# cbg-ethz/LongSom

Hardware: AMD Instinct MI355X
Metric: genomic sites/s pileup+call, 10M-read BAM x 5k barcodes, 1/2/4/8 MI355X (higher is better)
Workload: dtype u32

## Files before the change

longsom_amd/csrc/lsg_api.hip:

```cpp
#include "lsg_ctx.h"
#include <cstdarg>
#include <cstring>

namespace lsg {
static thread_local char g_err[512] = "";
void set_error(const char* fmt, ...) {
    va_list ap; va_start(ap, fmt); vsnprintf(g_err, sizeof(g_err), fmt, ap); va_end(ap);
}
const char* get_error() { return g_err; }

int run_count(lsg_ctx* c, const lsg_count_params* p);
int run_fetch_counts(lsg_ctx* c, int ct, int64_t* keys, uint8_t* ref, uint32_t* counts, int64_t capacity);
int run_call(lsg_ctx* c, const lsg_call_params* p);
int run_fetch_calls(lsg_ctx* c, lsg_call* out, int64_t capacity, int candidates_only, int64_t* n_out);
int run_select_calls(lsg_ctx* c, int kind, lsg_call* dst_device, int64_t capacity, int64_t* n_out);
int run_probe(lsg_ctx* c, const PosSet& s, const char* who, const int64_t* keys, int64_t n, uint8_t* hits, int on_device);
int run_step2_allele_queries(lsg_ctx* c, int64_t* keys_out, int64_t capacity, int64_t* n_out);
int run_set_table_names(lsg_ctx* c, int32_t n_contigs, const char* contig_names, int32_t n_ct, const char* ct_names);
int run_format_table(lsg_ctx* c, int32_t table, int64_t* n_bytes);
int run_copy_table(lsg_ctx* c, int32_t table, char* dst, int64_t capacity);
int run_append_table(lsg_ctx* c, int32_t table, const char* path);
int run_free_table(lsg_ctx* c, int32_t table);
int run_step2_summary(lsg_ctx* c, int32_t n_cols, uint8_t* kinds, int64_t* n_survivor_bytes);
int run_genotype(lsg_ctx* c, const lsg_genotype_params* p, int64_t n_sites, const int64_t* site_keys, const uint8_t* alt_sym,
                 uint32_t* dp, uint32_t* alt, int on_device, int32_t max_depth, int64_t n_groups, const int64_t* group_off);
int run_cellgeno_count(lsg_ctx* c, const lsg_genotype_params* p, int32_t max_depth, int64_t n_sites, const int64_t* site_keys, const uint8_t* alt_sym,
                       const uint8_t* is_chrm, int64_t n_groups, const int64_t* group_off, double alpha2, double beta2, double pvalue);
int run_cellgeno_load_counts(lsg_ctx* c, int64_t n_sites, int32_t n_cb, const uint32_t* dp, const uint32_t* alt, const uint8_t* is_chrm, double alpha2, double beta2, double pvalue);
int run_cellgeno_fetch(lsg_ctx* c, uint32_t* dp, uint32_t* alt, int32_t* vaf4, int32_t* p4, uint8_t* status, uint8_t* bin, int64_t* n_covered, int64_t* n_pass);
int run_cellgeno_set_text(lsg_ctx* c, const lsg_cellgeno_text* t);
int run_cellgeno_filter(lsg_ctx* c, int32_t min_cells_per_mut, int32_t min_pos_cov, const uint8_t* col_int_ok, int64_t* n_rows_kept, int32_t* n_cols_kept);
int run_cellgeno_filter_fetch(lsg_ctx* c, uint8_t* row_keep, uint8_t* col_keep, int32_t* row_mut, int32_t* col_cov_kept, int32_t* col_cov_all, uint8_t* col_int);
int run_cellgeno_load_cells(lsg_ctx* c, int64_t n_sites, int32_t n_cb, const uint8_t* bin, const int32_t* vaf4);
int run_format_cell_table(lsg_ctx* c, int32_t table, int64_t* n_bytes);
int run_bnpc_load(lsg_ctx* c, int64_t n_samples, int32_t n_cells, const int32_t* assign, int32_t k_max, int32_t n_muts, const float* params);
int run_bnpc_codist(lsg_ctx* c);
int run_bnpc_fetch_dist(lsg_ctx* c, uint32_t* out, int64_t capacity);
int run_bnpc_mpear(lsg_ctx* c, int32_t n_cuts, const int32_t* labels, uint64_t* same_pairs, uint64_t* same_sim, uint64_t* dist_sum);
int run_bnpc_mean_params(lsg_ctx* c, const int32_t* final_assign, int32_t n_clusters, double* params, uint8_t* branch, int32_t* n_used);
int run_bnpc_unload(lsg_ctx* c);
int run_bnpc_linkage(lsg_ctx* c, double* Z);
int run_bnpc_cut_tree(lsg_ctx* c, int32_t n_cuts, const int32_t* n_clusters, int32_t* labels);
int run_bnpc_cluster_counts(lsg_ctx* c, int64_t* sum_over_samples);
int run_sf4(lsg_ctx* c, int64_t items, const uint32_t* k, const uint32_t* n, double al, double be, int32_t* out, double* raw);

template <class T>
static int put(lsg_ctx* c, DevBuf& buf, const T*& dst, const T* src, int64_t n, int on_device, hipStream_t st = nullptr) {
    if (n <= 0 || !src) { dst = nullptr; return 0; }
    if (src == buf.as<T>()) { dst = src; return 0; }
    if (buf.reserve((size_t)n * sizeof(T))) return -1;
    LSG_HIP(hipMemcpyAsync(buf.p, src, (size_t)n * sizeof(T), on_device ? hipMemcpyDeviceToDevice : hipMemcpyHostToDevice, st ? st : c->stream));
    dst = buf.as<T>();
    return 0;
}
static int put_ref(lsg_ctx* c, DevBuf& buf, const uint8_t*& dst, const uint8_t* src, int64_t n, int on_device) {
    if (on_device) { dst = src; return 0; }
    if (buf.reserve((size_t)n)) return -1;
    LSG_HIP(hipMemcpyAsync(buf.p, src, (size_t)n, hipMemcpyHostToDevice, c->stream));
    dst = buf.as<uint8_t>();
    return 0;
}
}

using namespace lsg;

extern "C" {

const char* lsg_last_error(void) { return get_error(); }
const char* lsg_version(void) { return "longsom_hip 0.1 (gfx950)"; }

int lsg_create(int device_id, lsg_ctx** out) {
    if (!out) { set_error("lsg_create: out is NULL"); return -2; }
    *out = nullptr;
    int n = 0;
    if (hipGetDeviceCount(&n) != hipSuccess || n <= 0) {
        set_error("lsg_create: no HIP device visible (this library has no CPU fallback)");
        return -1;
    }
    if (device_id < 0 || device_id >= n) { set_error("lsg_create: device %d out of range [0,%d)", device_id, n); return -2; }
    LSG_HIP(hipSetDevice(device_id));
    lsg_ctx* c = new lsg_ctx();
    c->device = device_id;
    { hipDeviceProp_t prop; if (hipGetDeviceProperties(&prop, device_id) == hipSuccess && prop.multiProcessorCount > 0) c->n_cus = prop.multiProcessorCount; }
    if (hipStreamCreateWithFlags(&c->copy_stream, hipStreamNonBlocking) != hipSuccess || hipEventCreateWithFlags(&c->ev_copy, hipEventDisableTiming) != hipSuccess || hipEventCreateWithFlags(&c->ev_blk, hipEventDisableTiming) != hipSuccess || hipEventCreateWithFlags(&c->ev_lpt, hipEventDisableTiming) != hipSuccess ||
        hipStreamCreateWithFlags(&c->own_stream, hipStreamNonBlocking) != hipSuccess) {
        set_error("lsg_create: hipStreamCreate failed"); delete c; return -1;
    }
    c->stream = c->own_stream;
    if (hipHostMalloc(reinterpret_cast<void**>(&c->h_pin), 4096, hipHostMallocDefault) != hipSuccess) { set_error("lsg_create: hipHostMalloc failed"); delete c; return -1; }
    for (auto& e : c->ev)
        if (hipEventCreate(&e) != hipSuccess) { set_error("lsg_create: hipEventCreate failed"); delete c; return -1; }
    for (auto& e : c->evb)
        if (hipEventCreate(&e) != hipSuccess) { set_error("lsg_create: hipEventCreate failed"); delete c; return -1; }
    *out = c;
    return 0;
}

void lsg_destroy(lsg_ctx* c) {
    if (!c) return;
    (void)hipSetDevice(c->device);
    (void)hipStreamSynchronize(c->stream);
    DevBuf* bufs[] = {&c->d_tile_base, &c->d_contig_len, &c->d_ref_ptrs, &c->d_celltype_of, &c->d_ct_rank, &c->b_read_tid, &c->b_read_pos,
                      &c->b_read_flag, &c->b_read_mapq, &c->b_read_cb, &c->b_seg_read, &c->b_seg_start, &c->b_seg_len,
                      &c->b_seg_ev_off, &c->b_events, &c->d_read_key, &c->d_read_drop, &c->d_drop_pairs, &c->d_read_adm,
                      &c->d_ne_units, &c->d_ne_mask, &c->d_ne_rowbase, &c->d_ne_rowoff,
                      &c->d_scalars, &c->d_cub_tmp, &c->d_ix_stat, &c->d_tile_cap, &c->d_tile_off, &c->d_calls, &c->d_site_off, &c->d_tail_table, &c->d_pass_list, &c->d_defer_list, &c->d_xcd_queues};
    for (auto* b : bufs) b->release();
    for (auto& b : c->d_rows) b.release();
    for (auto& b : c->ref) b.release();
    for (auto& s : c->posset) s.keys.release();
    c->alleleset.keys.release();
    for (auto& b : c->syn) b.release();
    for (auto& b : c->gen) b.release();
    (void)run_free_table(c, -1);
    c->cg.release();
    c->bnpc.release();
    c->bnpcs.release();
    c->bb.release();
    c->tab_names.release();
    for (auto& b : c->ws) b.release();
    for (auto& b : c->tm) b.release();
    for (auto& b : c->bt) b.release();
    for (auto& e : c->ev) if (e) (void)hipEventDestroy(e);
    for (auto& e : c->evb) if (e) (void)hipEventDestroy(e);
    if (c->own_stream) (void)hipStreamDestroy(c->own_stream);
    if (c->copy_stream) (void)hipStreamDestroy(c->copy_stream);
    if (c->ev_copy) (void)hipEventDestroy(c->ev_copy);
    if (c->ev_blk) (void)hipEventDestroy(c->ev_blk);
    if (c->ev_lpt) (void)hipEventDestroy(c->ev_lpt);
    if (c->h_pin) (void)hipHostFree(c->h_pin);
    delete c;
}

int lsg_unload_reads(lsg_ctx* c) {
    if (!c) { set_error("lsg_unload_reads: NULL handle"); return -2; }
    LSG_HIP(hipSetDevice(c->device));
    LSG_HIP(hipStreamSynchronize(c->stream));
    DevBuf* bufs[] = {&c->b_read_tid, &c->b_read_pos, &c->b_read_flag, &c->b_read_mapq, &c->b_read_cb, &c->b_seg_read, &c->b_seg_start, &c->b_seg_len,
                      &c->b_seg_ev_off, &c->b_events, &c->d_read_key, &c->d_read_drop, &c->d_read_adm, &c->d_ne_units, &c->d_ne_mask, &c->d_ne_rowbase, &c->d_ne_rowoff,
                      &c->d_cub_tmp, &c->d_ix_stat, &c->d_tile_cap, &c->d_tile_off, &c->d_calls, &c->d_site_off, &c->d_pass_list, &c->d_defer_list};
    for (auto* b : bufs) b->release();
    for (auto& b : c->d_rows) b.release();
    for (auto& b : c->gen) b.release();
    for (auto& b : c->ws) b.release();
    for (auto& b : c->tm) b.release();
    for (auto& b : c->bt) b.release();
    c->rd = lsg_reads{};
    lsg::drop_store(c);
    c->row_cap = 0; c->n_ne = 0; c->n_columns = 0; c->n_sites = 0; c->n_cand = 0; c->n_pass = -1;
    for (auto& n : c->n_rows) n = 0;
    return 0;
}

int lsg_set_stream(lsg_ctx* c, void* hip_stream) {
    if (!c) { set_error("lsg_set_stream: NULL handle"); return -2; }
    (void)hipStreamSynchronize(c->stream);
    c->stream = hip_stream ? reinterpret_cast<hipStream_t>(hip_stream) : c->own_stream;
    return 0;
}

int lsg_synchronize(lsg_ctx* c) {
    if (!c) { set_error("lsg_synchronize: NULL handle"); return -2; }
    LSG_HIP(hipStreamSynchronize(c->stream));
    return 0;
}

int lsg_set_contigs(lsg_ctx* c, int32_t n_contigs, const int64_t* lengths) {
    if (!c || n_contigs <= 0 || !lengths) { set_error("lsg_set_contigs: bad arguments"); return -2; }
    LSG_HIP(hipSetDevice(c->device));
    c->n_contigs = n_contigs;
    c->tab_n_contigs = 0;
    c->contig_len.assign(lengths, lengths + n_contigs);
    c->tile_base.assign(n_contigs + 1, 0);
    uint64_t t = 0;
    for (int i = 0; i < n_contigs; ++i) {
        if (lengths[i] < 0 || lengths[i] > 0x7fffffffll) { set_error("lsg_set_contigs: contig %d length %lld unsupported", i, (long long)lengths[i]); return -2; }
        c->tile_base[i] = (uint32_t)t;
        t += (uint64_t)(((lengths[i] + TILE_W - 1) / TILE_W + 1) & ~1ll);
    }
    if (t * LSG_MAX_CELLTYPES >= 0x7fffffffull) { set_error("lsg_set_contigs: genome too large (%llu tiles)", (unsigned long long)t); return -2; }
    c->tile_base[n_contigs] = (uint32_t)t;
    c->n_tiles = (uint32_t)t;
    c->tile_lo = 0; c->tile_hi = (uint32_t)t;
    lsg::drop_store(c);
    c->rd = lsg_reads{};
    for (auto& b : c->ref) b.release();
    c->ref.assign(n_contigs, DevBuf());
    c->ref_ptr.assign(n_contigs, nullptr);
    if (c->d_tile_base.reserve((size_t)(n_contigs + 1) * 4) || c->d_contig_len.reserve((size_t)n_contigs * 8) ||
        c->d_ref_ptrs.reserve((size_t)n_contigs * sizeof(void*))) return -1;
    LSG_HIP(hipMemcpyAsync(c->d_tile_base.p, c->tile_base.data(), (size_t)(n_contigs + 1) * 4, hipMemcpyHostToDevice, c->stream));
    LSG_HIP(hipMemcpyAsync(c->d_contig_len.p, c->contig_len.data(), (size_t)n_contigs * 8, hipMemcpyHostToDevice, c->stream));
    LSG_HIP(hipMemsetAsync(c->d_ref_ptrs.p, 0, (size_t)n_contigs * sizeof(void*), c->stream));
    LSG_HIP(hipStreamSynchronize(c->stream));
    c->counted = c->called = false;
    return 0;
}

int lsg_load_reference(lsg_ctx* c, int32_t tid, const uint8_t* bases, int64_t len, int32_t on_device) {
    if (!c || !bases) { set_error("lsg_load_reference: bad arguments"); return -2; }
    if (tid < 0 || tid >= c->n_contigs) { set_error("lsg_load_reference: tid %d out of range", tid); return -2; }
    if (len != c->contig_len[tid]) { set_error("lsg_load_reference: contig %d has length %lld, got %lld bases", tid, (long long)c->contig_len[tid], (long long)len); return -2; }
    LSG_HIP(hipSetDevice(c->device));
    const uint8_t* p = nullptr;
    if (put_ref(c, c->ref[tid], p, bases, len > 0 ? len : 1, on_device)) return -1;
    c->ref_ptr[tid] = p;
    LSG_HIP(hipMemcpyAsync(c->d_ref_ptrs.as<const uint8_t*>() + tid, &c->ref_ptr[tid], sizeof(void*), hipMemcpyHostToDevice, c->stream));
    LSG_HIP(hipStreamSynchronize(c->stream));
    c->counted = c->called = false;
    return 0;
}

int lsg_set_barcodes(lsg_ctx* c, const uint8_t* celltype_of, int32_t n_cb, int32_t n_celltypes) {
    if (!c || !celltype_of || n_cb <= 0) { set_error("lsg_set_barcodes: bad arguments"); return -2; }
    if (n_celltypes <= 0 || n_celltypes > LSG_MAX_CELLTYPES) { set_error("lsg_set_barcodes: n_celltypes %d not in [1,%d]", n_celltypes, LSG_MAX_CELLTYPES); return -2; }
    if (n_cb > 0x00FFFFFF) { set_error("lsg_set_barcodes: more than 2^24-1 barcodes"); return -2; }
    LSG_HIP(hipSetDevice(c->device));
    if (c->n_cb == n_cb && c->n_ct == n_celltypes && c->h_celltype_of.size() == (size_t)n_cb && memcmp(c->h_celltype_of.data(), celltype_of, (size_t)n_cb) == 0) return 0;
    c->h_celltype_of.assign(celltype_of, celltype_of + n_cb);
    if (c->d_celltype_of.reserve((size_t)n_cb)) return -1;
    LSG_HIP(hipMemcpyAsync(c->d_celltype_of.p, celltype_of, (size_t)n_cb, hipMemcpyHostToDevice, c->stream));
    {
        std::vector<uint32_t> rank((size_t)n_cb, 0u);
        for (auto& v : c->ct_size) v = 0;
        for (int32_t i = 0; i < n_cb; ++i)
            if (celltype_of[i] < n_celltypes) rank[i] = c->ct_size[celltype_of[i]]++;
        if (c->d_ct_rank.reserve((size_t)n_cb * 4)) return -1;
        LSG_HIP(hipMemcpyAsync(c->d_ct_rank.p, rank.data(), (size_t)n_cb * 4, hipMemcpyHostToDevice, c->stream));
        LSG_HIP(hipStreamSynchronize(c->stream));
    }
    LSG_HIP(hipStreamSynchronize(c->stream));
    c->n_cb = n_cb; c->n_ct = n_celltypes;
    c->max_live_reads = -1; c->max_live_exact = -1;
    c->counted = c->called = false;
    return 0;
}

int lsg_set_keep_reads(lsg_ctx* c, int32_t keep) {
    if (!c) { set_error("lsg_set_keep_reads: NULL handle"); return -2; }
    c->keep_reads = keep != 0;
    return 0;
}

int lsg_set_events_layout(lsg_ctx* c, int32_t layout) {
    if (!c || (layout != LSG_LAYOUT_COMPACT && layout != LSG_LAYOUT_PHASED)) { set_error("lsg_set_events_layout: bad arguments"); return -2; }
    c->events_layout = layout;
    return 0;
}

int lsg_set_pileup_window(lsg_ctx* c, int32_t window) {
    if (!c || window < 64) { set_error("lsg_set_pileup_window: the window must be at least 64 positions"); return -2; }
    c->plp_window = window;
    return 0;
}

int lsg_set_count_at_load(lsg_ctx* c, const lsg_count_params* params) {
    if (!c) { set_error("lsg_set_count_at_load: NULL handle"); return -2; }
    c->cal_enabled = params != nullptr;
    if (params) c->cal_params = *params;
    return 0;
}

int lsg_set_keep_unlisted(lsg_ctx* c, int32_t on) {
    if (!c) { set_error("lsg_set_keep_unlisted: NULL handle"); return -2; }
    c->keep_unlisted = on != 0;
    return 0;
}

int lsg_set_split_filters(lsg_ctx* c, int32_t max_nm, int32_t max_nh, int32_t n_trim) {
    if (!c) { set_error("lsg_set_split_filters: NULL handle"); return -2; }
    if (n_trim < 0) { set_error("lsg_set_split_filters: n_trim %d < 0", (int)n_trim); return -2; }
    c->split_max_nm = max_nm < 0 ? -1 : max_nm; c->split_max_nh = max_nh < 0 ? -1 : max_nh; c->split_n_trim = n_trim;
    return 0;
}

int lsg_get_split_reasons(lsg_ctx* c, int64_t* n, int64_t* first_ordinal) {
    if (!c || !n || !first_ordinal) { set_error("lsg_get_split_reasons: bad arguments"); return -2; }
    for (int r = 0; r < 18; ++r) { n[r] = c->split_n[r]; first_ordinal[r] = c->split_first[r]; }
    return 0;
}

int lsg_set_store_policy(lsg_ctx* c, int32_t policy) {
    if (!c) { set_error("lsg_set_store_policy: NULL handle"); return -2; }
    if (policy != LSG_STORE_KEEP && policy != LSG_STORE_SKIP_WHEN_COUNTED) { set_error("lsg_set_store_policy: unknown policy %d", (int)policy); return -2; }
    c->store_policy = policy;
    return 0;
}

int lsg_set_load_filter(lsg_ctx* c, int32_t min_mq, uint32_t flag_exclude, int32_t ignore_orphans) {
    if (!c) { set_error("lsg_set_load_filter: NULL handle"); return -2; }
    c->lf_min_mq = min_mq; c->lf_flag_exclude = flag_exclude; c->lf_ignore_orphans = ignore_orphans ? 1 : 0;
    return 0;
}

static int check_load_filter(lsg_ctx* c, const char* who, int32_t min_mq, uint32_t flag_exclude, int32_t ignore_orphans) {
    if (min_mq < c->st_min_mq || (c->st_flag_exclude & ~flag_exclude) != 0 || (c->st_ignore_orphans && !ignore_orphans)) {
        set_error("%s: these read filters (min_mq %d, flag_exclude 0x%x, ignore_orphans %d) admit reads the load filter dropped (min_mq %d, flag_exclude 0x%x, ignore_orphans %d): "
                  "load the reads again under a filter no stricter than the counts' (lsg_set_load_filter)", who, min_mq, flag_exclude, ignore_orphans,
                  c->st_min_mq, c->st_flag_exclude, c->st_ignore_orphans);
        return -2;
    }
    return 0;
}

int lsg_load_reads(lsg_ctx* c, const lsg_reads* r) {
    if (!c || !r) { set_error("lsg_load_reads: bad arguments"); return -2; }
    if (c->n_contigs <= 0) { set_error("lsg_load_reads: set the contigs first (the store is laid out over their tiles)"); return -2; }
    if (r->n_reads < 0 || r->n_segs < 0 || r->n_events < 0) { set_error("lsg_load_reads: negative sizes"); return -2; }
    if (r->n_segs >= 0xFFFFFFF0ll || r->n_reads >= (1ll << 29)) { set_error("lsg_load_reads: more than 2^32 segments or 2^29 reads; load in windows"); return -2; }
    if (r->n_events >= (1ll << 40)) { set_error("lsg_load_reads: more than 2^40 events"); return -2; }
    LSG_HIP(hipSetDevice(c->device));
    lsg::drop_store(c);
    const lsg_reads in = *r;
    c->rd = lsg_reads{};
    c->rd.n_reads = in.n_reads; c->rd.n_segs = in.n_segs; c->rd.n_events = in.n_events; c->rd.on_device = 1;
    const int d = in.on_device;
    if (in.n_reads > 0 && (!in.read_tid || !in.read_flag || !in.read_mapq || !in.read_cb)) { c->rd = lsg_reads{}; set_error("lsg_load_reads: NULL read array"); return -2; }
    if (in.n_segs > 0 && (!in.seg_read || !in.seg_start || !in.seg_len || !in.seg_ev_off)) { c->rd = lsg_reads{}; set_error("lsg_load_reads: NULL segment array"); return -2; }
    if (in.n_events > 0 && !in.events) { c->rd = lsg_reads{}; set_error("lsg_load_reads: NULL events array"); return -2; }
    hipStream_t cs = nullptr;
    if (d && !c->keep_reads) {
        LSG_HIP(hipEventRecord(c->ev_copy, c->stream));
        LSG_HIP(hipStreamWaitEvent(c->copy_stream, c->ev_copy, 0));
        cs = c->copy_stream;
    }
    if (put(c, c->b_read_tid, c->rd.read_tid, in.read_tid, in.n_reads, d, cs) ||
        put(c, c->b_read_pos, c->rd.read_pos, in.read_pos, in.n_reads, d, cs) ||
        put(c, c->b_read_flag, c->rd.read_flag, in.read_flag, in.n_reads, d, cs) ||
        put(c, c->b_read_mapq, c->rd.read_mapq, in.read_mapq, in.n_reads, d, cs) ||
        put(c, c->b_read_cb, c->rd.read_cb, in.read_cb, in.n_reads, d, cs) ||
        put(c, c->b_seg_read, c->rd.seg_read, in.seg_read, in.n_segs, d, cs) ||
        put(c, c->b_seg_start, c->rd.seg_start, in.seg_start, in.n_segs, d, cs) ||
        put(c, c->b_seg_len, c->rd.seg_len, in.seg_len, in.n_segs, d, cs)) { if (cs) (void)hipStreamSynchronize(cs); c->rd = lsg_reads{}; return -1; }
    const uint16_t* ev = in.events; const int64_t* evo = in.seg_ev_off;
    const bool staged = !d || c->keep_reads;
    if (staged && (put(c, c->b_seg_ev_off, evo, in.seg_ev_off, in.n_segs, d) || put(c, c->b_events, ev, in.events, in.n_events, d))) { c->rd = lsg_reads{}; return -1; }
    if (staged && in.events && c->hint_phased_events == (const void*)in.events) c->hint_phased_events = ev;
    const int rc = lsg::build_store(c, ev, in.n_events, evo, cs ? &in : nullptr);
    if (cs) LSG_HIP(hipStreamSynchronize(cs));
    if (rc) { c->rd = lsg_reads{}; lsg::drop_store(c); return rc; }
    if (c->keep_reads) { c->rd.events = ev; c->rd.seg_ev_off = evo; }
    else { c->b_events.release(); c->b_seg_ev_off.release(); }
    return 0;
}

int lsg_set_region(lsg_ctx* c, int32_t tid_lo, int64_t pos_lo, int32_t tid_hi, int64_t pos_hi) {
    if (!c || c->n_contigs <= 0) { set_error("lsg_set_region: set contigs first"); return -2; }
    if (tid_lo < 0 || tid_lo > c->n_contigs || tid_hi < 0 || tid_hi > c->n_contigs || (pos_lo & 63) || (pos_hi & 63) || pos_lo < 0 || pos_hi < 0) {
        set_error("lsg_set_region: bad region (positions must be multiples of 64)"); return -2;
    }
    auto tile_of = [&](int32_t tid, int64_t pos) -> uint64_t {
        if (tid >= c->n_contigs) return c->n_tiles;
        uint64_t t = (uint64_t)c->tile_base[tid] + (uint64_t)(pos >> 6);
        return t < c->tile_base[tid + 1] ? t : c->tile_base[tid + 1];
    };
    uint64_t lo = tile_of(tid_lo, pos_lo), hi = tile_of(tid_hi, pos_hi);
    if (hi < lo) { set_error("lsg_set_region: empty or inverted region"); return -2; }
    if (c->tile_lo == (uint32_t)lo && c->tile_hi == (uint32_t)hi) return 0;
    c->tile_lo = (uint32_t)lo; c->tile_hi = (uint32_t)hi;
    c->counted = c->called = false;
    return 0;
}

int lsg_pileup_count(lsg_ctx* c, const lsg_count_params* params, int64_t* n_rows, int64_t* n_columns) {
    if (!c || !params) { set_error("lsg_pileup_count: bad arguments"); return -2; }
    LSG_HIP(hipSetDevice(c->device));
    if (int rc = check_load_filter(c, "lsg_pileup_count", params->min_mq, params->flag_exclude, params->ignore_orphans)) return rc;
    const bool have = c->counted && (c->counted_at_load || c->store_skipped) && memcmp(params, &c->last_params, sizeof(*params)) == 0;
    c->counted_at_load = false;
    if (!have) { int rc = run_count(c, params); if (rc) return rc; }
    if (n_rows) for (int i = 0; i < c->n_ct; ++i) n_rows[i] = c->n_rows[i];
    if (n_columns) *n_columns = c->n_columns;
    return 0;
}

int lsg_fetch_counts(lsg_ctx* c, int32_t ct, int64_t* keys, uint8_t* ref, uint32_t* counts, int64_t capacity) {
    if (!c || !keys || !ref || !counts) { set_error("lsg_fetch_counts: bad arguments"); return -2; }
    LSG_HIP(hipSetDevice(c->device));
    return run_fetch_counts(c, ct, keys, ref, counts, capacity);
}

int64_t lsg_max_live_reads(lsg_ctx* c) {
    if (!c) { set_error("lsg_max_live_reads: bad arguments"); return -1; }
    if (hipSetDevice(c->device) != hipSuccess) { set_error("lsg_max_live_reads: hipSetDevice failed"); return -1; }
    if (lsg::live_read_bound(c)) return -1;
    return c->max_live_reads;
}

int64_t lsg_max_live_reads_exact(lsg_ctx* c) {
    if (!c) { set_error("lsg_max_live_reads_exact: bad arguments"); return -1; }
    if (hipSetDevice(c->device) != hipSuccess) { set_error("lsg_max_live_reads_exact: hipSetDevice failed"); return -1; }
    if (lsg::live_read_bound_exact(c)) return -1;
    return c->max_live_exact;
}

int64_t lsg_max_live_reads_all(lsg_ctx* c) {
    if (!c) { set_error("lsg_max_live_reads_all: bad arguments"); return -1; }
    if (hipSetDevice(c->device) != hipSuccess) { set_error("lsg_max_live_reads_all: hipSetDevice failed"); return -1; }
    if (lsg::live_read_bound_all(c)) return -1;
    return c->max_live_all;
}

int lsg_get_store_shape(lsg_ctx* c, int64_t* n_entries, int64_t* n_blocks, int64_t* n_events) {
    if (!c) { set_error("lsg_get_store_shape: NULL handle"); return -2; }
    if (n_entries) *n_entries = (int64_t)c->tm_n;
    if (n_blocks) *n_blocks = (int64_t)c->tm_nblk;
    if (n_events) *n_events = c->tm_events;
    return 0;
}

int lsg_get_build_times(lsg_ctx* c, float* ms4) {
    if (!c || !ms4) { set_error("lsg_get_build_times: bad arguments"); return -2; }
    for (int i = 0; i < 4; ++i) ms4[i] = c->build_ms[i];
    return 0;
}

int lsg_get_count_stats(lsg_ctx* c, lsg_count_stats* out) {
    if (!c || !out) { set_error("lsg_get_count_stats: bad arguments"); return -2; }
    *out = c->stats;
    return 0;
}

int lsg_get_layout_info(lsg_ctx* c, int32_t* path, double* build_ms, int64_t* store_bytes) {
    if (!c) { set_error("lsg_get_layout_info: NULL handle"); return -2; }
    if (path) *path = c->store_skipped ? (c->wsh ? 6 : c->line_loads ? 5 : 4) : c->load_was_fused ? 3 : 2;
    if (build_ms) *build_ms = c->layout_build_ms;
    if (store_bytes) {
        int64_t b = 0;
        for (auto& x : c->tm) b += (int64_t)x.cap;
        for (auto& x : c->bt) b += (int64_t)x.cap;
        for (DevBuf* x : {&c->d_tile_cap, &c->d_tile_off, &c->b_events, &c->b_seg_ev_off, &c->b_read_tid, &c->b_read_pos, &c->b_read_flag, &c->b_read_mapq, &c->b_read_cb,
                          &c->b_seg_read, &c->b_seg_start, &c->b_seg_len}) b += (int64_t)x->cap;
        b += (int64_t)c->ws[WS_SEG_INFO].cap;
        *store_bytes = b;
    }
    return 0;
}

int lsg_call_step1(lsg_ctx* c, const lsg_call_params* params, int64_t* n_sites, int64_t* n_candidates) {
    if (!c || !params) { set_error("lsg_call_step1: bad arguments"); return -2; }
    LSG_HIP(hipSetDevice(c->device));
    int rc = run_call(c, params);
    if (rc) return rc;
    if (n_sites) *n_sites = c->n_sites;
    if (n_candidates) *n_candidates = c->n_cand;
    return 0;
}

int lsg_fetch_calls(lsg_ctx* c, lsg_call* out, int64_t capacity, int32_t candidates_only, int64_t* n_out) {
    if (!c || (!out && capacity > 0)) { set_error("lsg_fetch_calls: bad arguments"); return -2; }
    LSG_HIP(hipSetDevice(c->device));
    return run_fetch_calls(c, out, capacity, candidates_only, n_out);
}

int lsg_export_calls(lsg_ctx* c, int32_t kind, void* dst_device, int64_t capacity, int64_t* n_out) {
    if (!c || kind < 0 || kind > 2) { set_error("lsg_export_calls: bad arguments"); return -2; }
    LSG_HIP(hipSetDevice(c->device));
    return run_select_calls(c, kind, reinterpret_cast<lsg_call*>(dst_device), capacity, n_out);
}

int lsg_set_table_names(lsg_ctx* c, int32_t n_contigs, const char* contig_names, int32_t n_celltypes, const char* celltype_names) {
    if (!c || n_contigs < 0 || !contig_names || !celltype_names) { set_error("lsg_set_table_names: bad arguments"); return -2; }
    LSG_HIP(hipSetDevice(c->device));
    return run_set_table_names(c, n_contigs, contig_names, n_celltypes, celltype_names);
}
int lsg_format_table(lsg_ctx* c, int32_t table, int64_t* n_bytes) {
    if (!c) { set_error("lsg_format_table: bad arguments"); return -2; }
    LSG_HIP(hipSetDevice(c->device));
    if (table >= LSG_TABLE_CELL_LONG && table <= LSG_TABLE_BNPC_VAF) return run_format_cell_table(c, table, n_bytes);
    return run_format_table(c, table, n_bytes);
}
int lsg_copy_table(lsg_ctx* c, int32_t table, char* dst_host, int64_t capacity) {
    if (!c || (!dst_host && capacity > 0) || capacity < 0) { set_error("lsg_copy_table: bad arguments"); return -2; }
    LSG_HIP(hipSetDevice(c->device));
    return run_copy_table(c, table, dst_host, capacity);
}
int lsg_append_table(lsg_ctx* c, int32_t table, const char* path) {
    if (!c || !path || !*path) { set_error("lsg_append_table: bad arguments"); return -2; }
    return run_append_table(c, table, path);
}
int lsg_step2_summary(lsg_ctx* c, int32_t n_cols, uint8_t* kinds, int64_t* n_survivor_bytes) {
    if (!c || !kinds) { set_error("lsg_step2_summary: bad arguments"); return -2; }
    LSG_HIP(hipSetDevice(c->device));
    return run_step2_summary(c, n_cols, kinds, n_survivor_bytes);
}
int lsg_free_table(lsg_ctx* c, int32_t table) {
    if (!c) { set_error("lsg_free_table: bad arguments"); return -2; }
    LSG_HIP(hipSetDevice(c->device));
    return run_free_table(c, table);
}

int lsg_load_posset(lsg_ctx* c, int32_t kind, const int64_t* keys, int64_t n, int32_t on_device) {
    if (!c || kind < 0 || kind >= 3 || n < 0 || (n > 0 && !keys)) { set_error("lsg_load_posset: bad arguments"); return -2; }
    LSG_HIP(hipSetDevice(c->device));
    PosSet& s = c->posset[kind];
    s.n = 0;
    if (n == 0) return 0;
    if (s.keys.reserve((size_t)n * 8)) return -1;
    LSG_HIP(hipMemcpyAsync(s.keys.p, keys, (size_t)n * 8, on_device ? hipMemcpyDeviceToDevice : hipMemcpyHostToDevice, c->stream));
    LSG_HIP(hipStreamSynchronize(c->stream));
    s.n = n;
    return 0;
}

int lsg_probe_posset(lsg_ctx* c, int32_t kind, const int64_t* keys, int64_t n, uint8_t* hits, int32_t on_device) {
    if (!c || kind < 0 || kind >= 3 || n < 0 || (n > 0 && (!keys || !hits))) { set_error("lsg_probe_posset: bad arguments"); return -2; }
    LSG_HIP(hipSetDevice(c->device));
    return run_probe(c, c->posset[kind], "lsg_probe_posset", keys, n, hits, on_device);
}

int lsg_load_alleleset(lsg_ctx* c, const int64_t* keys, int64_t n, int32_t on_device) {
    if (!c || (n > 0 && !keys)) { set_error("lsg_load_alleleset: bad arguments"); return -2; }
    LSG_HIP(hipSetDevice(c->device));
    PosSet& s = c->alleleset;
    s.n = 0; c->alleleset_loaded = false;
    if (n < 0) return 0;
    if (n > 0) {
        if (s.keys.reserve((size_t)n * 8)) return -1;
        LSG_HIP(hipMemcpyAsync(s.keys.p, keys, (size_t)n * 8, on_device ? hipMemcpyDeviceToDevice : hipMemcpyHostToDevice, c->stream));
        LSG_HIP(hipStreamSynchronize(c->stream));
    }
    s.n = n; c->alleleset_loaded = true;
    return 0;
}

int lsg_probe_alleleset(lsg_ctx* c, const int64_t* keys, int64_t n, uint8_t* hits, int32_t on_device) {
    if (!c || n < 0 || (n > 0 && (!keys || !hits))) { set_error("lsg_probe_alleleset: bad arguments"); return -2; }
    if (!c->alleleset_loaded) { set_error("lsg_probe_alleleset: no allele set loaded (lsg_load_alleleset)"); return -2; }
    LSG_HIP(hipSetDevice(c->device));
    return run_probe(c, c->alleleset, "lsg_probe_alleleset", keys, n, hits, on_device);
}

int lsg_step2_allele_queries(lsg_ctx* c, int64_t* keys_out, int64_t capacity, int64_t* n) {
    if (!c || !n || capacity < 0 || (capacity > 0 && !keys_out)) { set_error("lsg_step2_allele_queries: bad arguments"); return -2; }
    LSG_HIP(hipSetDevice(c->device));
    return run_step2_allele_queries(c, keys_out, capacity, n);
}

int lsg_genotype_cells(lsg_ctx* c, const lsg_genotype_params* params, int64_t n_sites, const int64_t* site_keys,
                       const uint8_t* alt_sym, uint32_t* dp, uint32_t* alt, int32_t on_device) {
    if (!c || !params) { set_error("lsg_genotype_cells: bad arguments"); return -2; }
    LSG_HIP(hipSetDevice(c->device));
    if (int rc = check_load_filter(c, "lsg_genotype_cells", params->min_mq, params->flag_exclude, params->ignore_orphans)) return rc;
    return run_genotype(c, params, n_sites, site_keys, alt_sym, dp, alt, on_device, 0, 0, nullptr);
}

int lsg_genotype_cells_grouped(lsg_ctx* c, const lsg_genotype_params* params, int32_t max_depth, int64_t n_sites, const int64_t* site_keys, const uint8_t* alt_sym,
                               int64_t n_groups, const int64_t* group_off, uint32_t* dp, uint32_t* alt, int32_t on_device) {
    if (!c || !params || n_groups < 0 || (n_groups > 0 && !group_off)) { set_error("lsg_genotype_cells_grouped: bad arguments"); return -2; }
    LSG_HIP(hipSetDevice(c->device));
    if (int rc = check_load_filter(c, "lsg_genotype_cells_grouped", params->min_mq, params->flag_exclude, params->ignore_orphans)) return rc;
    if (n_groups > 0 && (group_off[0] != 0 || group_off[n_groups] != n_sites)) { set_error("lsg_genotype_cells_grouped: the groups must cover the sites"); return -2; }
    return run_genotype(c, params, n_sites, site_keys, alt_sym, dp, alt, on_device, max_depth, n_groups, group_off);
}

int lsg_cellgeno_count(lsg_ctx* c, const lsg_genotype_params* params, int32_t max_depth, int64_t n_sites, const int64_t* site_keys, const uint8_t* alt_sym,
                       const uint8_t* is_chrm, int64_t n_groups, const int64_t* group_off, double alpha2, double beta2, double pvalue) {
    if (!c || !params || n_sites < 0 || n_groups < 0 || (n_groups > 0 && !group_off) || (n_sites > 0 && (!site_keys || !alt_sym || !is_chrm))) { set_error("lsg_cellgeno_count: bad arguments"); return -2; }
    LSG_HIP(hipSetDevice(c->device));
    if (int rc = check_load_filter(c, "lsg_cellgeno_count", params->min_mq, params->flag_exclude, params->ignore_orphans)) return rc;
    if (n_groups > 0 && (group_off[0] != 0 || group_off[n_groups] != n_sites)) { set_error("lsg_cellgeno_count: the groups must cover the sites"); return -2; }
    return run_cellgeno_count(c, params, max_depth, n_sites, site_keys, alt_sym, is_chrm, n_groups, group_off, alpha2, beta2, pvalue);
}
int lsg_cellgeno_load_counts(lsg_ctx* c, int64_t n_sites, int32_t n_cb, const uint32_t* dp, const uint32_t* alt, const uint8_t* is_chrm, double alpha2, double beta2, double pvalue) {
    if (!c || n_sites < 0 || n_cb <= 0 || (n_sites > 0 && (!dp || !alt || !is_chrm))) { set_error("lsg_cellgeno_load_counts: bad arguments"); return -2; }
    LSG_HIP(hipSetDevice(c->device));
    return run_cellgeno_load_counts(c, n_sites, n_cb, dp, alt, is_chrm, alpha2, beta2, pvalue);
}
int lsg_cellgeno_fetch(lsg_ctx* c, uint32_t* dp, uint32_t* alt, int32_t* vaf4, int32_t* p4, uint8_t* status, uint8_t* bin, int64_t* n_covered, int64_t* n_pass) {
    if (!c) { set_error("lsg_cellgeno_fetch: NULL handle"); return -2; }
    LSG_HIP(hipSetDevice(c->device));
    return run_cellgeno_fetch(c, dp, alt, vaf4, p4, status, bin, n_covered, n_pass);
}
int lsg_cellgeno_set_text(lsg_ctx* c, const lsg_cellgeno_text* text) {
    if (!c || !text) { set_error("lsg_cellgeno_set_text: bad arguments"); return -2; }
    LSG_HIP(hipSetDevice(c->device));
    return run_cellgeno_set_text(c, text);
}
int lsg_cellgeno_filter(lsg_ctx* c, int32_t min_cells_per_mut, int32_t min_pos_cov, const uint8_t* col_int_ok, int64_t* n_rows_kept, int32_t* n_cols_kept) {
    if (!c) { set_error("lsg_cellgeno_filter: NULL handle"); return -2; }
    LSG_HIP(hipSetDevice(c->device));
    return run_cellgeno_filter(c, min_cells_per_mut, min_pos_cov, col_int_ok, n_rows_kept, n_cols_kept);
}
int lsg_cellgeno_filter_fetch(lsg_ctx* c, uint8_t* row_keep, uint8_t* col_keep, int32_t* row_mut, int32_t* col_cov_kept, int32_t* col_cov_all, uint8_t* col_int) {
    if (!c) { set_error("lsg_cellgeno_filter_fetch: NULL handle"); return -2; }
    LSG_HIP(hipSetDevice(c->device));
    return run_cellgeno_filter_fetch(c, row_keep, col_keep, row_mut, col_cov_kept, col_cov_all, col_int);
}
int lsg_cellgeno_load_cells(lsg_ctx* c, int64_t n_sites, int32_t n_cb, const uint8_t* bin, const int32_t* vaf4) {
    if (!c || n_sites < 0 || n_cb <= 0 || (n_sites > 0 && (!bin || !vaf4))) { set_error("lsg_cellgeno_load_cells: bad arguments"); return -2; }
    LSG_HIP(hipSetDevice(c->device));
    return run_cellgeno_load_cells(c, n_sites, n_cb, bin, vaf4);
}

int lsg_bnpc_load_samples(lsg_ctx* c, int64_t n_samples, int32_t n_cells, const int32_t* assign, int32_t k_max, int32_t n_muts, const float* params) {
    if (!c) { set_error("lsg_bnpc_load_samples: NULL handle"); return -2; }
    LSG_HIP(hipSetDevice(c->device));
    return run_bnpc_load(c, n_samples, n_cells, assign, k_max, n_muts, params);
}

int lsg_bnpc_codist(lsg_ctx* c) {
    if (!c) { set_error("lsg_bnpc_codist: NULL handle"); return -2; }
    LSG_HIP(hipSetDevice(c->device));
    return run_bnpc_codist(c);
}

int lsg_bnpc_fetch_dist(lsg_ctx* c, uint32_t* dist, int64_t capacity) {
    if (!c) { set_error("lsg_bnpc_fetch_dist: NULL handle"); return -2; }
    LSG_HIP(hipSetDevice(c->device));
    return run_bnpc_fetch_dist(c, dist, capacity);
}

int lsg_bnpc_mpear(lsg_ctx* c, int32_t n_cuts, const int32_t* labels, uint64_t* same_pairs, uint64_t* same_sim, uint64_t* dist_sum) {
    if (!c) { set_error("lsg_bnpc_mpear: NULL handle"); return -2; }
    LSG_HIP(hipSetDevice(c->device));
    return run_bnpc_mpear(c, n_cuts, labels, same_pairs, same_sim, dist_sum);
}

int lsg_bnpc_mean_params(lsg_ctx* c, const int32_t* final_assign, int32_t n_clusters, double* params, uint8_t* branch, int32_t* n_used) {
    if (!c) { set_error("lsg_bnpc_mean_params: NULL handle"); return -2; }
    LSG_HIP(hipSetDevice(c->device));
    return run_bnpc_mean_params(c, final_assign, n_clusters, params, branch, n_used);
}

int lsg_bnpc_linkage(lsg_ctx* c, double* Z) {
    if (!c) { set_error("lsg_bnpc_linkage: NULL handle"); return -2; }
    LSG_HIP(hipSetDevice(c->device));
    return run_bnpc_linkage(c, Z);
}

int lsg_bnpc_cut_tree(lsg_ctx* c, int32_t n_cuts, const int32_t* n_clusters, int32_t* labels) {
    if (!c) { set_error("lsg_bnpc_cut_tree: NULL handle"); return -2; }
    LSG_HIP(hipSetDevice(c->device));
    return run_bnpc_cut_tree(c, n_cuts, n_clusters, labels);
}

int lsg_bnpc_cluster_counts(lsg_ctx* c, int64_t* sum_over_samples) {
    if (!c) { set_error("lsg_bnpc_cluster_counts: NULL handle"); return -2; }
    LSG_HIP(hipSetDevice(c->device));
    return run_bnpc_cluster_counts(c, sum_over_samples);
}

int lsg_bnpc_unload(lsg_ctx* c) {
    if (!c) { set_error("lsg_bnpc_unload: NULL handle"); return -2; }
    LSG_HIP(hipSetDevice(c->device));
    return run_bnpc_unload(c);
}

int lsg_betabinom_sf4(lsg_ctx* c, int64_t n_items, const uint32_t* k, const uint32_t* n, double alpha, double beta, int32_t* out_p4) {
    if (!c) { set_error("lsg_betabinom_sf4: NULL handle"); return -2; }
    LSG_HIP(hipSetDevice(c->device));
    return run_sf4(c, n_items, k, n, alpha, beta, out_p4, nullptr);
}

int lsg_betabinom_sf(lsg_ctx* c, int64_t n_items, const uint32_t* k, const uint32_t* n, double alpha, double beta, int32_t* out_p4, double* out_p) {
    if (!c || !out_p) { set_error("lsg_betabinom_sf: bad arguments"); return -2; }
    LSG_HIP(hipSetDevice(c->device));
    return run_sf4(c, n_items, k, n, alpha, beta, out_p4, out_p);
}

}
```

longsom_amd/csrc/lsg_ctx.h:

```cpp
#pragma once
#include <hip/hip_runtime.h>
#include <cstdint>
#include <cstdio>
#include <string>
#include <vector>
#include "../../include/longsom_hip.h"
#include "../../include/longsom_synth.h"

namespace lsg {

constexpr int TILE_W = 64;
constexpr int ROW_PLANES = 34;
constexpr int NCTR = 33;

constexpr int ROW_QUADS = (ROW_PLANES + 3) / 4;
constexpr uint64_t ROW_BLOCK_WORDS = (uint64_t)ROW_QUADS * 256;
constexpr uint64_t ROW_STORED_WORDS = (uint64_t)ROW_QUADS * 4;
constexpr uint32_t ROW_NARROW = 1u << 31;
constexpr uint32_t ROW_NARROW_MAX = 256;
static_assert(ROW_NARROW_MAX * 255u < (1u << 16), "a narrow row's quality sum (two planes share a word) fits 16 bits");
__host__ __device__ inline uint64_t row_word(uint64_t row, int plane) {
    return (row >> 6) * ROW_BLOCK_WORDS + (uint64_t)(plane >> 2) * 256 + (row & 63) * 4 + (uint64_t)(plane & 3);
}

void set_error(const char* fmt, ...);
const char* get_error();

#define LSG_HIP(call)                                                                          \
    do {                                                                                       \
        hipError_t e_ = (call);                                                                \
        if (e_ != hipSuccess) {                                                                \
            lsg::set_error("%s failed: %s (%s:%d)", #call, hipGetErrorString(e_), __FILE__, __LINE__); \
            return -1;                                                                         \
        }                                                                                      \
    } while (0)

struct DevBuf {
    void* p = nullptr;
    size_t cap = 0;
    int reserve(size_t bytes) {
        if (bytes <= cap) return 0;
        if (p) { (void)hipFree(p); p = nullptr; cap = 0; }
        const size_t slack = bytes / 16 < ((size_t)64 << 20) ? bytes / 16 : ((size_t)64 << 20);
        size_t want = bytes + slack + 256;
        LSG_HIP(hipMalloc(&p, want));
        cap = want;
        return 0;
    }
    void release() { if (p) (void)hipFree(p); p = nullptr; cap = 0; }
    template <class T> T* as() const { return reinterpret_cast<T*>(p); }
};

struct PosSet { DevBuf keys; int64_t n = 0; };

struct CellGeno {
    DevBuf keys, alt_sym, is_chrm, dp, alt, vaf4, p4, status, bin, n_cov, n_pass, text, scratch, filt;
    int64_t n_sites = 0; int32_t n_cb = 0; bool valid = false;
    bool cells_only = false;
    bool text_valid = false; int64_t n_long = 0, n_mat = 0; int32_t n_cols = 0, float_cells = 0;
    size_t head_off_at = 0, index_off_at = 0, label_off_at = 0, cb_off_at = 0, ct_off_at = 0, long_order_at = 0, mat_order_at = 0, col_src_at = 0,
           head_at = 0, index_at = 0, label_at = 0, cb_at = 0, ct_at = 0;
    bool filt_valid = false; int64_t n_rows_kept = 0; int32_t n_cols_kept = 0;
    size_t f_row_mut_at = 0, f_cov_kept_at = 0, f_cov_all_at = 0, f_rows_at = 0, f_cols_at = 0, f_nsel_at = 0, f_row_keep_at = 0, f_col_keep_at = 0,
           f_col_int_at = 0, f_col_ok_at = 0;
    void release() { for (DevBuf* b : {&keys, &alt_sym, &is_chrm, &dp, &alt, &vaf4, &p4, &status, &bin, &n_cov, &n_pass, &text, &scratch, &filt}) b->release(); valid = text_valid = filt_valid = false; }
};

struct Bnpc {
    DevBuf lab, raw, params, dist, cuts, sums, rank, flags, owner, cl16, idx, mean, part, ord2, small;
    DevBuf work, wsmall, rec;
    std::vector<double> Z;
    std::vector<int32_t> cut_order;
    int64_t n_samples = 0; int32_t n_cells = 0, pitch = 0, k_max = 0, n_muts = 0;
    bool valid = false, dist_valid = false, has_params = false, tree_valid = false;
    void release() {
        for (DevBuf* b : {&lab, &raw, &params, &dist, &cuts, &sums, &rank, &flags, &owner, &cl16, &idx, &mean, &part, &ord2, &small, &work, &wsmall, &rec}) b->release();
        Z = {}; cut_order = {};
        valid = dist_valid = has_params = tree_valid = false;
    }
};

struct Bnpcs {
    DevBuf one, zero, pop, seeds, lab, size, colof, live, nlive, hi, theta, L1, L0, LL, alpha, prow, n1, n0, rowml, rowb, order, keys, rec_lab, rec_sc, arena, err;
    DevBuf sm_i, sm_d, sm_c, sm_t, rec_sm;
    DevBuf rates, rec_err, err_cnt, err_out;
    DevBuf psrf, psrf_out;
    DevBuf used;
    double err_prob = 0.0, err_prior[4] = {}, mix[2] = {};
    bool learn = false, fixed_assign = false;
    double sm_prob = 0.0, sm_ratio[2] = {0.75, 0.25};
    int32_t sm_scans = 3;
    int32_t n_cells = 0, n_muts = 0, n_words = 0, n_chains = 0, steps1 = 0, k_max = 0, ll_pitch = 0, pending = -1, next_step = 0;
    int32_t test_ml_end = 0;
    int64_t arena_rows = 0;
    double p = 1.0, q = 1.0, g0 = 0.0, g1 = 0.0, dpa_prob = 0.0, betaln = 0.0;
    bool valid = false, prepared = false;
    std::vector<int32_t> h_k;
    std::vector<int64_t> h_used;
    void release() {
        for (DevBuf* b : {&one, &zero, &pop, &seeds, &lab, &size, &colof, &live, &nlive, &hi, &theta, &L1, &L0, &LL, &alpha, &prow, &n1, &n0, &rowml, &rowb, &order, &keys, &rec_lab, &rec_sc,
                          &arena, &err, &sm_i, &sm_d, &sm_c, &sm_t, &rec_sm, &rates, &rec_err, &err_cnt, &err_out, &psrf, &psrf_out, &used}) b->release();
        valid = prepared = false;
    }
};

struct Bbfit {
    DevBuf hist, tails, out, ref, tmp;
    int64_t cap = 0;
    bool valid = false;
    void release() { for (DevBuf* b : {&hist, &tails, &out, &ref, &tmp}) b->release(); valid = false; cap = 0; }
};

enum { WS_NE_NSLOT = 0, WS_NE_ACC, WS_NE_GEOM, WS_MULTI_LIST, WS_MACC, WS_EXPORT_K, WS_EXPORT_R,
       WS_EXPORT_C, WS_CALL_FLAGS, WS_CALL_SEL, WS_CALL_CANDS, WS_CALL_TASKS, WS_SEG_INFO };

constexpr uint32_t CB_MASK = 0x00FFFFFFu;
constexpr uint32_t TM_RUNSTART = 1u << 31, TM_FWD = 1u << 30, TM_WHI = 1u << 29;
constexpr uint32_t TM_PAD_S0 = CB_MASK | TM_RUNSTART;
constexpr int TM_GROUP = 4;
enum { TM_STORE = 0, TM_S0, TM_B, TM_RD, TM_META, TM_BLK_TILE, TM_BLK_OFF, TM_EXT,
       TM_JOBS, TM_NE_UNITS, TM_NE_GEOM, TM_NE_NSLOT, TM_NE_ACC, TM_MULTI, TM_CHUNKS, TM_NBUF };
struct TmJob { uint32_t e0, e1, w0, slab, nj, cnt, tile, emid, base, off; int32_t tstart, tid; };
constexpr int TM_JOB_WORDS = 12;
static_assert(sizeof(TmJob) == 4 * TM_JOB_WORDS, "TmJob layout");
constexpr uint32_t TMJ_WIDE = 1u << 31;
constexpr int TM_JOB_TGT = 3072, TM_JOB_LIMIT = 4095;

}

struct lsg_ctx;
namespace lsg {
int build_store(lsg_ctx* c, const uint16_t* events, int64_t n_events, const int64_t* seg_ev_off, const lsg_reads* src = nullptr);
int ensure_plan(lsg_ctx* c);
void drop_store(lsg_ctx* c);
int live_read_bound(lsg_ctx* c);
int live_read_bound_exact(lsg_ctx* c);
int live_read_bound_all(lsg_ctx* c);
__global__ void k_read_end(const uint32_t* seg_read, const int32_t* seg_start, const int32_t* seg_len, int64_t n_segs, int32_t* read_end);
__global__ void k_read_end_init(const int32_t* read_pos, int64_t n_reads, int32_t* read_end);
int depth_cap_drops(lsg_ctx* c, const lsg_count_params* p);
struct GatherCountSrc { const uint16_t* events; int64_t n_events; const uint64_t* key; const uint32_t* rdv; int32_t cb_bits; int32_t src_shift; int32_t wsh; };
int unit_row_offsets(lsg_ctx* c, int ct, const uint32_t** off);
int run_gather_count(lsg_ctx* c, const lsg_count_params* p, const GatherCountSrc& src, bool direct);
}

struct lsg_ctx {
    int device = 0;
    hipStream_t stream = nullptr;
    hipStream_t own_stream = nullptr;
    hipStream_t copy_stream = nullptr;
    hipEvent_t ev_copy = nullptr;
    hipEvent_t ev_blk = nullptr;
    hipEvent_t ev_lpt = nullptr;
    hipEvent_t ev[6] = {nullptr, nullptr, nullptr, nullptr, nullptr, nullptr};
    hipEvent_t evb[5] = {nullptr, nullptr, nullptr, nullptr, nullptr};

    int32_t n_contigs = 0;
    std::vector<int64_t> contig_len;
    std::vector<uint32_t> tile_base;
    uint32_t n_tiles = 0;
    uint32_t tile_lo = 0, tile_hi = 0;
    lsg::DevBuf d_tile_base, d_contig_len, d_ref_ptrs;
    std::vector<lsg::DevBuf> ref;
    std::vector<const uint8_t*> ref_ptr;

    int32_t n_cb = 0, n_ct = 0;
    lsg::DevBuf d_celltype_of, d_ct_rank;
    std::vector<uint8_t> h_celltype_of;
    uint32_t ct_size[LSG_MAX_CELLTYPES] = {0, 0, 0, 0};

    lsg_reads rd{};
    lsg::DevBuf b_read_tid, b_read_pos, b_read_flag, b_read_mapq, b_read_cb;
    lsg::DevBuf b_seg_read, b_seg_start, b_seg_len, b_seg_ev_off, b_events;
    int32_t plp_window = 50000, st_window = 50000;
    int32_t lf_min_mq = 0, lf_ignore_orphans = 0; uint32_t lf_flag_exclude = 0;
    int32_t st_min_mq = 0, st_ignore_orphans = 0; uint32_t st_flag_exclude = 0;
    bool keep_unlisted = false;
    int32_t split_max_nm = -1, split_max_nh = -1, split_n_trim = 0;
    int64_t split_n[18] = {}, split_first[18] = {};
    bool keep_reads = false;
    lsg::DevBuf d_tile_cap, d_tile_off;
    lsg::DevBuf tm[lsg::TM_NBUF];
    lsg::DevBuf bt[18];
    uint64_t tm_n = 0;
    int64_t tm_events = 0;
    uint64_t tm_np = 0;
    uint32_t tm_nblk = 0, tm_njobs = 0, tm_nchunks = 0, tm_n_ne = 0, tm_n_multi = 0, tm_n_slabs = 0, tm_n_wide = 0;
    int plan_n_ct = 0;
    int plan1_n_ct = 0;
    uint32_t plan1_tot[4] = {0, 0, 0, 0};
    uint32_t plan_misc[2] = {0, 0};
    uint32_t* d_plan_misc = nullptr;
    bool cal_enabled = false; lsg_count_params cal_params{};
    bool counted_at_load = false;
    bool load_was_fused = false;
    bool tm_valid = false;
    int32_t store_policy = 0;
    bool store_skipped = false;
    double layout_build_ms = 0;
    float build_ms[4] = {0, 0, 0, 0};
    int64_t max_live_reads = -1;
    int64_t max_live_all = -1;
    int32_t wsh = 0;
    int32_t events_layout = 0;
    const void* hint_phased_events = nullptr;
    bool src_phased = false;
    bool line_loads = false;
    int64_t max_live_exact = -1;
    lsg::DevBuf d_read_drop;
    lsg::DevBuf d_drop_pairs; int64_t n_drop_pairs = 0;
    lsg::DevBuf d_read_adm;
    bool has_drops = false;
    int64_t n_depth_dropped = 0;

    lsg::DevBuf d_read_key;
    lsg::DevBuf d_ne_units, d_ne_mask, d_ne_rowbase, d_ne_rowoff, d_scalars, d_cub_tmp, d_ix_stat;
    lsg::DevBuf d_rows[LSG_MAX_CELLTYPES];
    uint64_t row_cap = 0;
    uint32_t arena = 256;
    uint32_t n_ne = 0;
    int64_t n_rows[LSG_MAX_CELLTYPES] = {0, 0, 0, 0};
    int64_t n_columns = 0;
    lsg_count_params last_params{};
    lsg_count_stats stats{};
    bool counted = false;

    lsg::DevBuf d_calls, d_site_off, d_tail_table;
    double tail_table_key[4] = {0, 0, 0, 0}; bool tail_table_valid = false;
    int64_t n_sites = 0, n_cand = 0, n_pass = -1;
    lsg::DevBuf d_pass_list, d_defer_list, d_xcd_queues;
    uint32_t call_tasks_per_site = 1;
    bool called = false;

    lsg::DevBuf tab_keys[LSG_MAX_CELLTYPES], tab_refs[LSG_MAX_CELLTYPES], tab_rows[LSG_MAX_CELLTYPES], tab_names, tab_scratch, tab_scratch2;
    int32_t tab_scratch_table = -1; int64_t tab_scratch_rows = 0;
    uint64_t tab_rows_serial[LSG_MAX_CELLTYPES] = {0, 0, 0, 0};
    uint64_t count_serial = 0;
    lsg::DevBuf tab_text[LSG_TABLE_SLOTS];
    int64_t tab_bytes[LSG_TABLE_SLOTS];
    lsg_ctx() { for (auto& b : tab_bytes) b = -1; }
    int32_t tab_n_contigs = 0, tab_n_ct = 0; uint32_t tab_ct_off_at = 0, tab_order_at = 0, tab_ct_txt_at = 0, tab_contig_txt_at = 0;

    lsg::CellGeno cg;

    lsg::Bnpc bnpc;
    lsg::Bnpcs bnpcs;
    lsg::Bbfit bb;

    lsg::PosSet posset[3];
    lsg::PosSet alleleset; bool alleleset_loaded = false;
    lsg::DevBuf syn[12];
    lsg::DevBuf gen[10];
    lsg::DevBuf ws[16];
    int n_cus = 256;
    unsigned long long* h_pin = nullptr;
    uint32_t n_multi = 0;
};
```

longsom_amd/csrc/store.hip:

```cpp
#include "lsg_ctx.h"
#include <hipcub/hipcub.hpp>
#include <chrono>
#include <cstdio>
#include <cstdlib>
#include <utility>

namespace lsg {

constexpr uint32_t KEY_INVALID = 0xFFFFFFFFu;

constexpr uint32_t RV_WHI = 1u << 29, RV_SEGFIRST = 1u << 30, RV_FWD = 1u << 31, RV_READ = RV_WHI - 1u;
__host__ __device__ __forceinline__ uint64_t sort_key(uint32_t cb, uint32_t first, uint32_t nev1, uint64_t src, int cb_bits, int wsh = 0) {
    return (uint64_t)cb | ((uint64_t)(first | (nev1 << (6 + wsh))) << cb_bits) | (src << (cb_bits + 12 + 2 * wsh));
}

struct BuildArgs {
    int64_t n_reads, n_segs, n_events;
    const int32_t* read_tid; const uint16_t* read_flag; const uint8_t* read_mapq; const int32_t* read_cb;
    const uint32_t* seg_read; const int32_t* seg_start; const int32_t* seg_len; const int64_t* seg_ev_off;
    const uint32_t* tile_base; const int64_t* contig_len;
    int32_t n_contigs; uint32_t n_tiles;
    uint2* seg_info;
    uint32_t* tile_cap;
    uint32_t* cursor;
    uint64_t* key; uint32_t* rdv;
    int32_t cb_bits;
    unsigned long long* qhead;
    int32_t lf_min_mq, lf_ignore_orphans; uint32_t lf_flag_exclude;
    uint32_t* bad;
    unsigned long long* n_ev;
    int32_t* span_diff;
    int32_t* cap_diff;
    int32_t window;
    int32_t wsh;
    int32_t src_shift;
};

__device__ __forceinline__ int64_t win_edge_after(int64_t x, int32_t W) { return 1 + (int64_t)W * (int64_t)((x >= 1 ? (uint32_t)(x - 1) / (uint32_t)W : 0u) + 1u); }
__device__ __forceinline__ int64_t win_edge_in_tile(int64_t tstart, int32_t W) {
    const int64_t b = win_edge_after(tstart, W);
    return b < tstart + TILE_W ? b : -1;
}

constexpr int SEG_THREADS = 256, SEG_U = 4, SEG_H = 2048, SEG_MAX_SINCE = 6;
__global__ __launch_bounds__(SEG_THREADS) void k_seg_static(BuildArgs a) {
    __shared__ uint32_t hkey[SEG_H];
    __shared__ int32_t hval[SEG_H];
    __shared__ unsigned long long s_ev;
    __shared__ uint32_t s_new, s_flush;
    for (int i = threadIdx.x; i < SEG_H; i += SEG_THREADS) { hkey[i] = KEY_INVALID; hval[i] = 0; }
    if (threadIdx.x == 0) { s_ev = 0; s_new = 0; s_flush = 0; }
    auto slot = [&](uint32_t t) -> int {
        uint32_t h = (t * 2654435761u) >> 21;
        for (int tries = 0; tries < 16; ++tries) {
            const uint32_t prev = atomicCAS(&hkey[h], KEY_INVALID, t);
            if (prev == KEY_INVALID) { atomicAdd(&s_new, 1u); return (int)h; }
            if (prev == t) return (int)h;
            h = (h + 1) & (SEG_H - 1);
        }
        return -1;
    };
    auto mark = [&](uint32_t t, int32_t v) { const int h = slot(t); if (h >= 0) atomicAdd(&hval[h], v); else atomicAdd(a.span_diff + t, v); };
    auto mark_cap = [&](uint32_t t, int32_t v) { const int h = slot(t); if (h >= 0) atomicAdd(&hval[h], v * 65536); else atomicAdd(a.cap_diff + t, v); };
    unsigned long long n_ev = 0;
    bool unphased = false;
    constexpr int64_t BATCH = (int64_t)SEG_THREADS * SEG_U;
    const int64_t n_batches = (a.n_segs + BATCH - 1) / BATCH;
    const int64_t per_wg = (n_batches + gridDim.x - 1) / gridDim.x;
    const int64_t b_lo = (int64_t)blockIdx.x * per_wg, b_hi = b_lo + per_wg < n_batches ? b_lo + per_wg : n_batches;
    const int64_t last_seg = a.n_segs - 1;
    int since = 0;
    __syncthreads();
    for (int64_t bt = b_lo; bt < b_hi; ++bt) {
        int64_t sg[SEG_U], st_[SEG_U], ln_[SEG_U], of_[SEG_U]; uint32_t rd_[SEG_U], rp_[SEG_U], rn_[SEG_U]; bool in_[SEG_U];
#pragma unroll
        for (int u = 0; u < SEG_U; ++u) {
            sg[u] = bt * BATCH + (int64_t)u * SEG_THREADS + threadIdx.x;
            in_[u] = sg[u] < a.n_segs;
            const int64_t si = in_[u] ? sg[u] : last_seg;
            rd_[u] = a.seg_read[si]; st_[u] = a.seg_start[si]; ln_[u] = a.seg_len[si]; of_[u] = a.seg_ev_off[si];
            rp_[u] = a.seg_read[si > 0 ? si - 1 : 0]; rn_[u] = a.seg_read[si < last_seg ? si + 1 : last_seg];
        }
        int32_t tid_[SEG_U], cb_[SEG_U]; uint32_t flag_[SEG_U], mq_[SEG_U];
#pragma unroll
        for (int u = 0; u < SEG_U; ++u) {
            const int64_t ri = (int64_t)rd_[u] < a.n_reads ? (int64_t)rd_[u] : 0;
            tid_[u] = a.read_tid[ri]; cb_[u] = a.read_cb[ri]; flag_[u] = a.read_flag[ri]; mq_[u] = (uint32_t)a.read_mapq[ri];
        }
        int64_t clen_[SEG_U]; uint32_t tb_[SEG_U], te_[SEG_U];
#pragma unroll
        for (int u = 0; u < SEG_U; ++u) {
            const int ti = tid_[u] >= 0 && tid_[u] < a.n_contigs ? tid_[u] : 0;
            clen_[u] = a.contig_len[ti]; tb_[u] = a.tile_base[ti]; te_[u] = a.tile_base[ti + 1];
        }
#pragma unroll
        for (int u = 0; u < SEG_U; ++u) {
        const int64_t s = sg[u];
        uint32_t edge_tile = KEY_INVALID;
        if (in_[u]) {
            const uint32_t r = rd_[u];
            uint32_t key = KEY_INVALID, tb = 0;
            if ((int64_t)r >= a.n_reads) atomicOr(a.bad, 2u);
            else {
                const int64_t st = st_[u], ln = ln_[u], o = of_[u];
                const int32_t tid = tid_[u], cb = cb_[u];
                const bool on_contig = tid >= 0 && tid < a.n_contigs;
                if (ln > 0 && (o < 0 || o + ln > a.n_events)) atomicOr(a.bad, 1u);
                else {
                    const uint32_t flag = flag_[u];
                    bool pool = (int)mq_[u] >= a.lf_min_mq && (flag & a.lf_flag_exclude) == 0;
                    if (pool && a.lf_ignore_orphans && (flag & 1u) && !(flag & 2u)) pool = false;
                    if (pool && on_contig && cb >= 0 && (uint32_t)cb < CB_MASK && !(st < 0 || ln <= 0 || st + ln > clen_[u])) {
                        key = (uint32_t)cb | (((flag >> 4) & 1u) << 24);
                        tb = tb_[u];
                        n_ev += (unsigned long long)ln;
                        unphased |= ((o - st) & (int64_t)((64 << a.wsh) - 1)) != 0;
                        mark_cap((tb + ((uint32_t)st >> 6)) >> a.wsh, 1);
                        mark_cap(((tb + ((uint32_t)(st + ln - 1) >> 6)) >> a.wsh) + 1, -1);
                        int nb = 0;
                        for (int64_t b = win_edge_after(st, a.window); b < st + ln; b += a.window) {
                            if ((b & (int64_t)((64 << a.wsh) - 1)) == 0) continue;
                            const uint32_t t = (tb + (uint32_t)(b >> 6)) >> a.wsh;
                            if (nb++ == 0) edge_tile = t;
                            else { atomicAdd(a.cap_diff + t, 1); atomicAdd(a.cap_diff + t + 1, -1); }
                        }
                    }
                }
                if (a.span_diff && on_contig && cb >= 0) {
                    const bool first = s == 0 || rp_[u] != r, last = s + 1 == a.n_segs || rn_[u] != r;
                    const uint32_t t0 = tb_[u], te = te_[u];
                    if ((first || last) && te > t0) {
                        int64_t b = st < 0 ? 0 : st, e = st + (ln > 0 ? ln : 0);
                        if (e < 0) e = 0;
                        if (first) { uint32_t t = t0 + (uint32_t)(b >> 6); if (t >= te) t = te - 1; mark(t >> a.wsh, 1); }
                        if (last) { uint32_t t = t0 + (uint32_t)(e >> 6); if (t >= te) t = te - 1; mark((t >> a.wsh) + 1, -1); }
                    }
                }
            }
            a.seg_info[s] = make_uint2(key, tb);
        }
        for (unsigned long long todo = __ballot(edge_tile != KEY_INVALID); todo;) {
            const uint32_t lt = (uint32_t)__shfl((int)edge_tile, __ffsll((long long)todo) - 1);
            const unsigned long long same = __ballot(edge_tile == lt);
            if ((threadIdx.x & 63) == (unsigned)(__ffsll((long long)todo) - 1)) { const int n = __popcll(same); atomicAdd(a.cap_diff + lt, n); atomicAdd(a.cap_diff + lt + 1, -n); }
            todo &= ~same;
        }
        }
        ++since;
        __syncthreads();
        if (threadIdx.x == 0) {
            s_flush = (bt + 1 == b_hi || s_new > SEG_H / 2 || since >= SEG_MAX_SINCE) ? 1u : 0u;
            if (s_flush) s_new = 0;
        }
        __syncthreads();
        if (s_flush) {
            since = 0;
            for (int i = threadIdx.x; i < SEG_H; i += SEG_THREADS)
                if (hkey[i] != KEY_INVALID) {
                    const int32_t w = hval[i], v = (int32_t)(int16_t)(w & 0xffff), cp = (w - v) >> 16;
                    if (v != 0) atomicAdd(a.span_diff + hkey[i], v);
                    if (cp != 0) atomicAdd(a.cap_diff + hkey[i], cp);
                    hkey[i] = KEY_INVALID; hval[i] = 0;
                }
            __syncthreads();
        }
    }
    for (int o = 32; o > 0; o >>= 1) n_ev += __shfl_down(n_ev, o);
    __syncthreads();
    if ((threadIdx.x & 63) == 0 && n_ev) atomicAdd(&s_ev, n_ev);
    __syncthreads();
    if (threadIdx.x == 0 && s_ev) atomicAdd(a.n_ev, s_ev);
    if (__syncthreads_or(unphased ? 1 : 0) && threadIdx.x == 0) atomicOr(a.bad, 4u);
}

constexpr int BIN_THREADS = 256;
constexpr int BIN_TPR = 8;
constexpr int BIN_H = 4096;
constexpr int BIN_SUPER = 16;
constexpr int BIN_MAXI = 32;
constexpr uint32_t BIN_FILL = BIN_H * 5 / 8;

template <class OP>
__device__ __forceinline__ uint32_t wave_reduce_last(uint32_t v, OP op) {
    v = op(v, (uint32_t)__builtin_amdgcn_update_dpp(0, (int)v, 0x111, 0xf, 0xf, true));
    v = op(v, (uint32_t)__builtin_amdgcn_update_dpp(0, (int)v, 0x112, 0xf, 0xf, true));
    v = op(v, (uint32_t)__builtin_amdgcn_update_dpp(0, (int)v, 0x114, 0xf, 0xf, true));
    v = op(v, (uint32_t)__builtin_amdgcn_update_dpp(0, (int)v, 0x118, 0xf, 0xf, true));
    v = op(v, (uint32_t)__builtin_amdgcn_update_dpp(0, (int)v, 0x142, 0xa, 0xf, false));
    v = op(v, (uint32_t)__builtin_amdgcn_update_dpp(0, (int)v, 0x143, 0xc, 0xf, false));
    return v;
}
struct BinSeg { uint32_t key, tb, t0, rd; int32_t st, ln, ntile; int64_t evoff, b1; };

struct BinRaw { uint2 info; int32_t st, ln; int64_t evoff; uint32_t rd; };
__device__ __forceinline__ BinRaw bin_fetch(const BuildArgs& a, int64_t s) {
    const int64_t si = s < a.n_segs ? s : a.n_segs - 1;
    BinRaw w;
    w.info = a.seg_info[si]; w.st = a.seg_start[si]; w.ln = a.seg_len[si]; w.evoff = a.seg_ev_off[si]; w.rd = a.seg_read[si];
    return w;
}
template <bool FULL>
__device__ __forceinline__ BinSeg bin_make(const BuildArgs& a, int64_t s, const BinRaw& w) {
    BinSeg g; g.key = KEY_INVALID; g.tb = 0; g.t0 = 0; g.rd = 0; g.b1 = 0; g.st = 0; g.ln = 0; g.ntile = 0; g.evoff = 0;
    if (FULL) asm volatile("" :: "v"(w.info.x), "v"(w.info.y), "v"(w.st), "v"(w.ln), "v"(w.evoff), "v"(w.rd));
    else asm volatile("" :: "v"(w.info.x), "v"(w.info.y), "v"(w.st), "v"(w.ln));
    const uint2 info = w.info;
    const int bs = 6 + a.wsh;
    if (s < a.n_segs && info.x != KEY_INVALID) {
        g.key = info.x; g.tb = info.y >> a.wsh;
        g.st = w.st; g.ln = w.ln; g.evoff = w.evoff; g.rd = w.rd;
        g.t0 = g.tb + ((uint32_t)g.st >> bs);
        g.ntile = (int)(((uint32_t)(g.st + g.ln - 1) >> bs) - ((uint32_t)g.st >> bs)) + 1;
        g.b1 = win_edge_after(g.st, a.window);
        for (int64_t b = g.b1; b < (int64_t)g.st + g.ln; b += a.window) g.ntile += (b & (int64_t)((1 << bs) - 1)) != 0;
    } else if (s < a.n_segs) g.tb = info.y >> a.wsh;
    return g;
}
__device__ __forceinline__ void bin_piece(const BinSeg& g, int32_t W, int bs, int k, uint32_t& tile_rel, int32_t& lo, int32_t& hi) {
    const int32_t en = g.st + g.ln;
    const int64_t bmask = (int64_t)((1 << bs) - 1);
    int shift = 0;
    int64_t b = g.b1;
    for (; b < en; b += W) {
        if ((b & bmask) == 0) continue;
        const int idx = (int)((b >> bs) - (g.st >> bs)) + shift + 1;
        if (k < idx) break;
        if (k == idx) {
            tile_rel = (uint32_t)((b >> bs) - (g.st >> bs)); lo = (int32_t)b;
            const int32_t tend = (int32_t)(((b >> bs) + 1) << bs);
            hi = en < tend ? en : tend;
            return;
        }
        ++shift;
    }
    tile_rel = (uint32_t)(k - shift);
    const int32_t tstart = (int32_t)((((uint32_t)g.st >> bs) + tile_rel) << bs);
    lo = g.st > tstart ? g.st : tstart;
    hi = en < tstart + (1 << bs) ? en : tstart + (1 << bs);
    if (b < hi && b > lo && (b & bmask) != 0) hi = (int32_t)b;
}

__global__ __launch_bounds__(BIN_THREADS) void k_bin(BuildArgs a) {
    __shared__ uint32_t hkey[BIN_H], hcnt[BIN_H];
    __shared__ uint32_t s_newb[BIN_MAXI], s_ib[BIN_MAXI], s_ir[BIN_MAXI];
    __shared__ int s_maxb[BIN_MAXI];
    __shared__ uint32_t s_super;
    const int t = threadIdx.x, lane = t & 63;
    constexpr int HSHIFT = 32 - __builtin_ctz(BIN_H);
    for (int i = t; i < BIN_H; i += BIN_THREADS) { hkey[i] = KEY_INVALID; hcnt[i] = 0; }
    const int64_t n_batches = (a.n_segs + BIN_THREADS - 1) / BIN_THREADS;
    const int64_t n_super = (n_batches + BIN_SUPER - 1) / BIN_SUPER;
    for (bool first = true;; first = false) {
        __syncthreads();
        if (t == 0) s_super = first ? blockIdx.x : (uint32_t)atomicAdd(a.qhead, 1ull) + gridDim.x;
        __syncthreads();
        const int64_t sup = (uint32_t)__builtin_amdgcn_readfirstlane((int)s_super);
        if (sup >= n_super) break;
        const int64_t b0 = sup * BIN_SUPER;
        const int64_t b1 = b0 + BIN_SUPER < n_batches ? b0 + BIN_SUPER : n_batches;
        int64_t cb = b0; int cr = 0;
        BinRaw nx = bin_fetch(a, cb * BIN_THREADS + t);
        while (cb < b1) {
            if (t < BIN_MAXI) { s_newb[t] = 0; s_maxb[t] = 0; }
            __syncthreads();
            int ni = 0; uint32_t tot = 0;
            int64_t b = cb; int r = cr;
            bool stop = false;
            while (!stop && b < b1) {
                const BinSeg g = bin_make<false>(a, b * BIN_THREADS + t, nx);
                nx = bin_fetch(a, (b + 1 < b1 ? b + 1 : b) * BIN_THREADS + t);
                const int ni_first = ni;
                const int wmax = (int)wave_reduce_last((uint32_t)g.ntile, [](uint32_t x, uint32_t y) { return x > y ? x : y; });
                if (lane == 63 && wmax) atomicMax(&s_maxb[ni_first], wmax);
                int R = -1;
                for (;;) {
                    uint32_t newc = 0;
                    uint32_t x[BIN_TPR], h[BIN_TPR], prev[BIN_TPR];
#pragma unroll
                    for (int j = 0; j < BIN_TPR; ++j) {
                        const int k = r * BIN_TPR + j;
                        x[j] = KEY_INVALID; h[j] = 0; prev[j] = 0;
                        if (k < g.ntile) {
                            uint32_t trel; int32_t lo_, hi_;
                            bin_piece(g, a.window, 6 + a.wsh, k, trel, lo_, hi_);
                            x[j] = g.t0 + trel;
                            h[j] = (x[j] * 2654435761u) >> HSHIFT;
                        }
                    }
#pragma unroll
                    for (int j = 0; j < BIN_TPR; ++j)
                        if (x[j] != KEY_INVALID) prev[j] = atomicCAS(&hkey[h[j]], KEY_INVALID, x[j]);
#pragma unroll
                    for (int j = 0; j < BIN_TPR; ++j)
                        if (x[j] != KEY_INVALID) {
                            uint32_t hh = h[j], p = prev[j];
                            if (p == KEY_INVALID) ++newc;
                            else
                                while (p != x[j]) {
                                    hh = (hh + 1) & (BIN_H - 1);
                                    p = atomicCAS(&hkey[hh], KEY_INVALID, x[j]);
                                    if (p == KEY_INVALID) { ++newc; break; }
                                }
                            atomicAdd(&hcnt[hh], 1u);
                        }
                    newc = wave_reduce_last(newc, [](uint32_t x, uint32_t y) { return x + y; });
                    if (lane == 63 && newc) atomicAdd(&s_newb[ni], newc);
                    if (t == 0) { s_ib[ni] = (uint32_t)(b - b0); s_ir[ni] = (uint32_t)r; }
                    __syncthreads();
                    if (R < 0) R = __builtin_amdgcn_readfirstlane((s_maxb[ni_first] + BIN_TPR - 1) / BIN_TPR);
                    tot += (uint32_t)__builtin_amdgcn_readfirstlane((int)s_newb[ni]);
                    ++ni; ++r;
                    if (r >= R) { ++b; r = 0; }
                    if (ni >= BIN_MAXI || tot + BIN_THREADS * BIN_TPR > BIN_FILL) { stop = true; break; }
                    if (r == 0) break;
                }
            }
            nx = bin_fetch(a, cb * BIN_THREADS + t);
            for (int i = t; i < BIN_H; i += BIN_THREADS) {
                const uint32_t cnt = hcnt[i];
                if (cnt) hcnt[i] = atomicAdd(&a.cursor[hkey[i]], cnt);
            }
            __syncthreads();
            {
                const uint32_t ibl = (uint32_t)__builtin_amdgcn_readfirstlane((int)s_ib[ni - 1]);
                const int64_t b_next = b < b1 ? b : b1 - 1;
                uint32_t ib = (uint32_t)(cb - b0);
                BinSeg g = bin_make<true>(a, cb * BIN_THREADS + t, nx);
                nx = bin_fetch(a, (ib < ibl ? b0 + ib + 1 : b_next) * BIN_THREADS + t);
                for (int it = 0; it < ni; ++it) {
                    const int rr = __builtin_amdgcn_readfirstlane((int)s_ir[it]);
                    const uint32_t nb = it + 1 < ni ? (uint32_t)__builtin_amdgcn_readfirstlane((int)s_ib[it + 1]) : ib;
                    uint32_t x_[BIN_TPR], h_[BIN_TPR], hk_[BIN_TPR], pos_[BIN_TPR]; int32_t lo_[BIN_TPR], hi_[BIN_TPR];
#pragma unroll
                    for (int j = 0; j < BIN_TPR; ++j) {
                        const int k = rr * BIN_TPR + j;
                        x_[j] = KEY_INVALID; h_[j] = 0; hk_[j] = KEY_INVALID; pos_[j] = 0; lo_[j] = 0; hi_[j] = 0;
                        if (k < g.ntile) {
                            uint32_t trel;
                            bin_piece(g, a.window, 6 + a.wsh, k, trel, lo_[j], hi_[j]);
                            x_[j] = g.t0 + trel;
                            h_[j] = (x_[j] * 2654435761u) >> HSHIFT;
                            hk_[j] = hkey[h_[j]];
                        }
                    }
#pragma unroll
                    for (int j = 0; j < BIN_TPR; ++j)
                        if (x_[j] != KEY_INVALID) {
                            while (hk_[j] != x_[j]) { h_[j] = (h_[j] + 1) & (BIN_H - 1); hk_[j] = hkey[h_[j]]; }
                            pos_[j] = atomicAdd(&hcnt[h_[j]], 1u);
                        }
                    BinSeg gn = g;
                    if (nb != ib) {
                        gn = bin_make<true>(a, (b0 + nb) * BIN_THREADS + t, nx);
                        nx = bin_fetch(a, (nb < ibl ? b0 + nb + 1 : b_next) * BIN_THREADS + t);
                    }
#pragma unroll
                    for (int j = 0; j < BIN_TPR; ++j) {
                        if (x_[j] != KEY_INVALID) {
                            const uint32_t x = x_[j]; const int32_t lo = lo_[j], hi = hi_[j];
                            const uint32_t pos = pos_[j];
                            const int32_t tstart = (int32_t)((x - g.tb) << (6 + a.wsh));
                            int64_t edge = -1;
                            { int64_t e = g.b1 - a.window; while (e + a.window <= lo) e += a.window; if (e > tstart && e <= lo && e > 1) edge = e; }
                            const uint64_t src = (uint64_t)(g.evoff + (lo - g.st)) >> a.src_shift;
                            const uint64_t key = sort_key(g.key & CB_MASK, (uint32_t)(lo - tstart), (uint32_t)(hi - lo - 1), src, a.cb_bits, a.wsh);
                            const uint32_t flags = (lo == g.st ? RV_SEGFIRST : 0u) | (((g.key >> 24) & 1u) ? 0u : RV_FWD);
                            if (a.rdv) { a.key[pos] = key; a.rdv[pos] = g.rd | flags | (edge >= 0 && lo >= edge ? RV_WHI : 0u); }
                            else a.key[pos] = key | ((uint64_t)flags << 32);
                        }
                    }
                    g = gn; ib = nb;
                }
                __syncthreads();
                for (int i = t; i < BIN_H; i += BIN_THREADS)
                    if (hkey[i] != KEY_INVALID) { hkey[i] = KEY_INVALID; hcnt[i] = 0; }
            }
            cb = b; cr = r;
        }
    }
}

constexpr int TT_THREADS = 256, TT_SUB = TT_THREADS * 4, TT_MAX_CHUNKS = 1024;
struct TtAgg1 { int32_t d, s, smax, pad; };
struct TtAgg2 { unsigned long long c; uint32_t b, ne; };
struct TtArgs {
    const int32_t* cap_diff; const int32_t* span_diff; uint32_t T; uint32_t chunk;
    uint32_t n_chunks;
    TtAgg1* agg1; int32_t* din; TtAgg2* agg2; TtAgg2* in2;
    uint32_t* cap; uint32_t* tile_off; uint32_t* blk_off; uint32_t* netile;
    uint32_t* d_small; unsigned long long* d_sum;
};
template <int NT, class V>
__device__ __forceinline__ V tt_wg_exscan(V v, V& total, V* sh ) {
    const int lane = threadIdx.x & 63, wv = threadIdx.x >> 6;
    V inc = v;
    for (int o = 1; o < 64; o <<= 1) { const V u = __shfl_up(inc, o); if (lane >= o) inc += u; }
    __syncthreads();
    if (lane == 63) sh[wv] = inc;
    __syncthreads();
    V base = 0, tot = 0;
    for (int w = 0; w < NT / 64; ++w) { const V x = sh[w]; if (w < wv) base += x; tot += x; }
    total = tot;
    return base + inc - v;
}
__global__ __launch_bounds__(TT_THREADS) void k_tt_marks(TtArgs a) {
    __shared__ int32_t sh[TT_THREADS / 64 + 1];
    __shared__ int32_t sh_max[TT_THREADS / 64];
    const uint32_t lo = blockIdx.x * a.chunk, hi = lo + a.chunk < a.T + 1 ? lo + a.chunk : a.T + 1;
    int32_t dsum = 0, srun = 0, smax = INT32_MIN;
    for (uint32_t b0 = lo; b0 < hi; b0 += TT_SUB) {
        const uint32_t i0 = b0 + threadIdx.x * 4;
        int32_t d[4], sp[4];
#pragma unroll
        for (int k = 0; k < 4; ++k) { const bool in = i0 + k < hi; d[k] = in ? a.cap_diff[i0 + k] : 0; sp[k] = in && a.span_diff ? a.span_diff[i0 + k] : 0; }
        int32_t ds = d[0] + d[1] + d[2] + d[3];
        int32_t r = 0, m = INT32_MIN;
#pragma unroll
        for (int k = 0; k < 4; ++k) { r += sp[k]; if (i0 + k < hi) m = r > m ? r : m; }
        int32_t tot_s; const int32_t ex = tt_wg_exscan<TT_THREADS>(r, tot_s, sh);
        if (m != INT32_MIN) { const int32_t v = srun + ex + m; smax = v > smax ? v : smax; }
        srun += tot_s; dsum += ds;
    }
    for (int o = 32; o > 0; o >>= 1) { const int32_t u = __shfl_down(smax, o); smax = u > smax ? u : smax; dsum += __shfl_down(dsum, o); }
    __syncthreads();
    if ((threadIdx.x & 63) == 0) { sh_max[threadIdx.x >> 6] = smax; sh[threadIdx.x >> 6] = dsum; }
    __syncthreads();
    if (threadIdx.x == 0) {
        int32_t m = INT32_MIN, dd = 0;
        for (int w = 0; w < TT_THREADS / 64; ++w) { m = sh_max[w] > m ? sh_max[w] : m; dd += sh[w]; }
        a.agg1[blockIdx.x] = TtAgg1{dd, srun, m, 0};
    }
}
__global__ __launch_bounds__(TT_MAX_CHUNKS) void k_tt_scan1(TtArgs a) {
    __shared__ int32_t sh[TT_MAX_CHUNKS / 64 + 1];
    __shared__ int32_t sh_max[TT_MAX_CHUNKS / 64];
    const uint32_t i = threadIdx.x;
    TtAgg1 g{0, 0, INT32_MIN, 0};
    if (i < a.n_chunks) g = a.agg1[i];
    int32_t tot;
    const int32_t din = tt_wg_exscan<TT_MAX_CHUNKS>(g.d, tot, sh);
    const int32_t sin = tt_wg_exscan<TT_MAX_CHUNKS>(g.s, tot, sh);
    if (i < a.n_chunks) a.din[i] = din;
    int32_t m = i < a.n_chunks && g.smax != INT32_MIN ? sin + g.smax : INT32_MIN;
    for (int o = 32; o > 0; o >>= 1) { const int32_t u = __shfl_down(m, o); m = u > m ? u : m; }
    __syncthreads();
    if ((i & 63) == 0) sh_max[i >> 6] = m;
    __syncthreads();
    if (i == 0) { int32_t mm = INT32_MIN; for (int w = 0; w < TT_MAX_CHUNKS / 64; ++w) mm = sh_max[w] > mm ? sh_max[w] : mm; a.d_small[3] = (uint32_t)mm; }
}
__global__ __launch_bounds__(TT_THREADS) void k_tt_caps(TtArgs a) {
    __shared__ int32_t sh[TT_THREADS / 64 + 1];
    __shared__ unsigned long long sh_c[TT_THREADS / 64];
    __shared__ uint32_t sh_b[TT_THREADS / 64], sh_n[TT_THREADS / 64];
    const uint32_t lo = blockIdx.x * a.chunk, hi = lo + a.chunk < a.T + 1 ? lo + a.chunk : a.T + 1;
    int32_t run = a.din[blockIdx.x];
    unsigned long long csum = 0; uint32_t bsum = 0, nsum = 0;
    for (uint32_t b0 = lo; b0 < hi; b0 += TT_SUB) {
        const uint32_t i0 = b0 + threadIdx.x * 4;
        int32_t d[4];
#pragma unroll
        for (int k = 0; k < 4; ++k) d[k] = i0 + k < hi ? a.cap_diff[i0 + k] : 0;
        int32_t tot; const int32_t ex = tt_wg_exscan<TT_THREADS>(d[0] + d[1] + d[2] + d[3], tot, sh);
        int32_t r = run + ex;
#pragma unroll
        for (int k = 0; k < 4; ++k) {
            r += d[k];
            if (i0 + k < hi) {
                a.cap[i0 + k] = (uint32_t)r;
                if (i0 + k < a.T) { const uint32_t cv = (uint32_t)r; csum += cv; bsum += (cv + 7u) / 8u; nsum += cv != 0u; }
            }
        }
        run += tot;
    }
    for (int o = 32; o > 0; o >>= 1) { csum += __shfl_down(csum, o); bsum += __shfl_down(bsum, o); nsum += __shfl_down(nsum, o); }
    __syncthreads();
    if ((threadIdx.x & 63) == 0) { sh_c[threadIdx.x >> 6] = csum; sh_b[threadIdx.x >> 6] = bsum; sh_n[threadIdx.x >> 6] = nsum; }
    __syncthreads();
    if (threadIdx.x == 0) {
        TtAgg2 g{0, 0, 0};
        for (int w = 0; w < TT_THREADS / 64; ++w) { g.c += sh_c[w]; g.b += sh_b[w]; g.ne += sh_n[w]; }
        a.agg2[blockIdx.x] = g;
    }
}
__global__ __launch_bounds__(TT_MAX_CHUNKS) void k_tt_scan2(TtArgs a) {
    __shared__ unsigned long long sh64[TT_MAX_CHUNKS / 64 + 1];
    __shared__ uint32_t sh32[TT_MAX_CHUNKS / 64 + 1];
    const uint32_t i = threadIdx.x;
    TtAgg2 g{0, 0, 0};
    if (i < a.n_chunks) g = a.agg2[i];
    unsigned long long tc; uint32_t tb, tn;
    TtAgg2 in;
    in.c = tt_wg_exscan<TT_MAX_CHUNKS>(g.c, tc, sh64);
    in.b = tt_wg_exscan<TT_MAX_CHUNKS>(g.b, tb, sh32);
    in.ne = tt_wg_exscan<TT_MAX_CHUNKS>(g.ne, tn, sh32);
    if (i < a.n_chunks) a.in2[i] = in;
    if (i == 0) { *a.d_sum = tc; a.d_small[1] = tn; }
}
__global__ __launch_bounds__(TT_THREADS) void k_tt_offsets(TtArgs a) {
    __shared__ uint32_t sh[TT_THREADS / 64 + 1];
    const uint32_t lo = blockIdx.x * a.chunk, hi = lo + a.chunk < a.T + 1 ? lo + a.chunk : a.T + 1;
    const TtAgg2 in = a.in2[blockIdx.x];
    uint32_t crun = (uint32_t)in.c, brun = in.b, nrun = in.ne;
    for (uint32_t b0 = lo; b0 < hi; b0 += TT_SUB) {
        const uint32_t i0 = b0 + threadIdx.x * 4;
        uint32_t cv[4], bv[4], nv[4];
#pragma unroll
        for (int k = 0; k < 4; ++k) { cv[k] = i0 + k < hi && i0 + k < a.T ? a.cap[i0 + k] : 0u; bv[k] = (cv[k] + 7u) / 8u; nv[k] = cv[k] != 0u; }
        uint32_t tc, tb, tn;
        uint32_t ec = crun + tt_wg_exscan<TT_THREADS>(cv[0] + cv[1] + cv[2] + cv[3], tc, sh);
        uint32_t eb = brun + tt_wg_exscan<TT_THREADS>(bv[0] + bv[1] + bv[2] + bv[3], tb, sh);
        uint32_t en = nrun + tt_wg_exscan<TT_THREADS>(nv[0] + nv[1] + nv[2] + nv[3], tn, sh);
#pragma unroll
        for (int k = 0; k < 4; ++k) {
            if (i0 + k < hi) {
                a.tile_off[i0 + k] = ec; a.blk_off[i0 + k] = eb;
                if (nv[k]) a.netile[en] = i0 + k;
            }
            ec += cv[k]; eb += bv[k]; en += nv[k];
        }
        crun += tc; brun += tb; nrun += tn;
    }
}
constexpr uint32_t SORT_LARGE = 256;
__global__ void k_seg_bounds(const uint32_t* netile, uint32_t n, const uint32_t* tile_off, uint32_t* begin, uint32_t* end, uint32_t* begin2, uint32_t* end2) {
    const uint32_t i = blockIdx.x * blockDim.x + threadIdx.x;
    if (i >= n) return;
    const uint32_t t = netile[i], b = tile_off[t], e = tile_off[t + 1];
    const bool large = e - b > SORT_LARGE;
    begin[i] = b; end[i] = large ? e : b;
    begin2[i] = b; end2[i] = large ? b : e;
}
__global__ void k_tile_caps(const uint32_t* tiles, uint32_t n, const uint32_t* cap, uint32_t* out) {
    const uint32_t i = blockIdx.x * blockDim.x + threadIdx.x;
    if (i < n) out[i] = cap[tiles[i]] >> 11;
}
__global__ void k_tm_blk_mark(const uint32_t* cap, const uint32_t* blk_off, uint32_t n_tiles, uint32_t* blk_tile) {
    const uint32_t t = blockIdx.x * blockDim.x + threadIdx.x;
    if (t < n_tiles && cap[t]) blk_tile[blk_off[t]] = t;
}

constexpr int TMG_BLOCKS = 4, TMG_WAVES = 4;
typedef uint32_t u32x4 __attribute__((ext_vector_type(4)));
struct __attribute__((packed, aligned(2))) U4A2 { u32x4 v; };
__global__ __launch_bounds__(TMG_WAVES * 64) void k_tm_gather(const uint16_t* events, int64_t n_events, const uint64_t* key, const uint32_t* rdv, int cb_bits, int src_shift,
                                                               const uint32_t* tile_off, const uint32_t* blk_off, const uint32_t* blk_tile, uint32_t nblk,
                                                               uint32_t* s0, uint8_t* b8, uint32_t* rd, uint4* store, uint16_t* ext) {
    __shared__ __attribute__((aligned(16))) uint16_t lds[TMG_WAVES][TMG_BLOCKS][8][64];
    const int lane = threadIdx.x & 63, wv = threadIdx.x >> 6;
    const uint32_t per_xcd = gridDim.x >> 3;
    const uint32_t vwg = (blockIdx.x & 7u) * per_xcd + (blockIdx.x >> 3);
    const uint32_t blk0 = (vwg * TMG_WAVES + (uint32_t)wv) * TMG_BLOCKS;
    if (blk0 >= nblk) return;
    uint32_t e_src = 0, e_info = 0;
    if (lane < 8 * TMG_BLOCKS) {
        const uint32_t blk = blk0 + ((uint32_t)lane >> 3);
        if (blk < nblk) {
            const uint64_t p = (uint64_t)blk * 8 + (lane & 7);
            const uint32_t t = blk_tile[blk];
            const uint32_t i = (uint32_t)(p - (uint64_t)blk_off[t] * 8), off = tile_off[t], n = tile_off[t + 1] - off;
            auto put = [](auto* q, auto v) { __builtin_nontemporal_store(v, q); };
            if (i >= n) { put(s0 + p, (uint32_t)TM_PAD_S0); put(b8 + p, (uint8_t)0); put(rd + p, 0u); }
            else {
                const uint32_t j = off + i, cbm = (1u << cb_bits) - 1u;
                const uint64_t k64 = key[j];
                const uint32_t k = (uint32_t)k64 & cbm, v = rdv[j];
                const bool rs = i == 0 || ((uint32_t)key[j - 1] & cbm) != k;
                const bool single = rs && (i + 1 == n || ((uint32_t)key[j + 1] & cbm) != k);
                const uint32_t geom = (uint32_t)(k64 >> cb_bits), first = geom & 63u, nev1 = (geom >> 6) & 63u;
                const uint64_t src = ((k64 >> (cb_bits + 12)) << src_shift) | (src_shift ? first : 0u);
                put(s0 + p, k | ((v & RV_FWD) ? TM_FWD : 0u) | ((v & RV_WHI) ? TM_WHI : 0u) | (rs ? TM_RUNSTART : 0u));
                put(b8 + p, (uint8_t)(nev1 | ((v & RV_SEGFIRST) ? 64u : 0u) | (single ? 128u : 0u)));
                put(rd + p, v & RV_READ);
                e_src = (uint32_t)src; e_info = (uint32_t)(src >> 32) | (first << 8) | ((nev1 + 1u) << 16);
            }
        }
    }
    const int u = lane >> 3, c = lane & 7;
    u32x4 chunk[TMG_BLOCKS];
    uint32_t info[TMG_BLOCKS];
#pragma unroll
    for (int q = 0; q < TMG_BLOCKS; ++q) {
        chunk[q] = u32x4{0u, 0u, 0u, 0u};
        const uint32_t lo32 = (uint32_t)__shfl((int)e_src, q * 8 + u), inf = (uint32_t)__shfl((int)e_info, q * 8 + u);
        info[q] = inf;
        const uint32_t nev = inf >> 16;
        if ((uint32_t)c * 8u < nev) {
            const int64_t off = (int64_t)(((uint64_t)(inf & 0xffu) << 32) | lo32) + c * 8;
            if (off + 8 <= n_events) chunk[q] = reinterpret_cast<const U4A2*>(events + off)->v;
            else {
                uint32_t w[4] = {0u, 0u, 0u, 0u};
                for (int i = 0; i < 8; ++i) if (off + i < n_events) w[i >> 1] |= (uint32_t)events[off + i] << (16 * (i & 1));
                chunk[q] = u32x4{w[0], w[1], w[2], w[3]};
            }
        }
    }
#pragma unroll
    for (int q = 0; q < TMG_BLOCKS; ++q) *reinterpret_cast<u32x4*>(&lds[wv][q][u][c * 8]) = chunk[q];
    __builtin_amdgcn_fence(__ATOMIC_ACQ_REL, "workgroup");
    __builtin_amdgcn_wave_barrier();
#pragma unroll
    for (int q = 0; q < TMG_BLOCKS; ++q) {
        const uint32_t blk = blk0 + q;
        if (blk >= nblk) break;
        uint32_t e[8], any = 0;
#pragma unroll
        for (int uu = 0; uu < 8; ++uu) {
            const uint32_t inf = (uint32_t)__builtin_amdgcn_readlane((int)info[q], uu * 8);
            const uint32_t idx = (uint32_t)lane - ((inf >> 8) & 63u);
            e[uu] = idx < (inf >> 16) ? (uint32_t)lds[wv][q][uu][idx & 63u] : 0u;
            any |= e[uu];
        }
        const unsigned long long m = __ballot(any != 0u);
        const int first = m ? __ffsll((long long)m) - 1 : 0, last = m ? 64 - __clzll((long long)m) : 0;
        if (lane >= first && lane < last) {
            const u32x4 row = {e[0] | (e[1] << 16), e[2] | (e[3] << 16), e[4] | (e[5] << 16), e[6] | (e[7] << 16)};
            u32x4* dst = reinterpret_cast<u32x4*>(store) + (uint64_t)blk * 64 + lane;
            __builtin_nontemporal_store(row, dst);
        }
        if (lane == 0) ext[blk] = (uint16_t)(first | (last << 8));
    }
}

#define SCAN_U32(in, out, n)                                                                              \
    do {                                                                                                  \
        size_t tb_ = 0;                                                                                   \
        LSG_HIP(hipcub::DeviceScan::ExclusiveSum(nullptr, tb_, (in), (out), (int)(n), st));              \
        if (c->d_cub_tmp.reserve(tb_ + 256)) return -1;                                                   \
        tb_ = c->d_cub_tmp.cap;                                                                           \
        LSG_HIP(hipcub::DeviceScan::ExclusiveSum(c->d_cub_tmp.p, tb_, (in), (out), (int)(n), st));       \
    } while (0)

enum { BT_KEY_A = 0, BT_KEY_B, BT_VAL_A, BT_VAL_B, BT_PEX, BT_NETILE, BT_SEG_BEGIN, BT_SEG_END, BT_TMP, BT_PER_TILE, BT_OFFS, BT_SPAN, BT_CURSOR, BT_LPT, BT_COPY_TMP, BT_N };

void drop_store(lsg_ctx* c) {
    c->tm_valid = false; c->plan_n_ct = 0; c->plan1_n_ct = 0; c->tm_n = 0; c->tm_events = 0; c->tm_np = 0; c->tm_nblk = 0; c->tm_njobs = 0; c->tm_nchunks = 0;
    c->tm_n_ne = 0; c->tm_n_multi = 0; c->tm_n_slabs = 0; c->tm_n_wide = 0;
    c->max_live_reads = -1; c->max_live_all = -1; c->max_live_exact = -1; c->has_drops = false;
    c->counted = c->called = false; c->counted_at_load = false; c->load_was_fused = false; c->store_skipped = false;
}

static void settle_temporaries(lsg_ctx* c) {
    size_t held = 0, mem_free = 0, mem_total = 0;
    for (auto& b : c->bt) held += b.cap;
    held += c->ws[WS_SEG_INFO].cap;
    if (hipMemGetInfo(&mem_free, &mem_total) != hipSuccess) return;
    const bool tight = c->store_skipped ? mem_free < mem_total / 4 : (held > mem_total / 8 || mem_free < mem_total / 8);
    if (tight) { for (auto& b : c->bt) b.release(); c->ws[WS_SEG_INFO].release(); c->plan1_n_ct = 0; }
}

static int plan_tiles(lsg_ctx* c, hipStream_t st);
static int plan_jobs(lsg_ctx* c, bool finish, const uint64_t* skey = nullptr, int cb_bits = 0);
static void plan_finish(lsg_ctx* c);
static void plan_finish_tiles(lsg_ctx* c);

template <unsigned RB, unsigned BS = 256, unsigned IPT = 8>
using LsgSortConfig = rocprim::segmented_radix_sort_config<RB, rocprim::kernel_config<BS, IPT>, rocprim::WarpSortConfig<16, 4, 256, 64, 32, 8, 256>>;
template <unsigned RB, unsigned BS, unsigned IPT, class... Args>
static hipError_t lsg_segmented_sort(Args&&... args) { return rocprim::segmented_radix_sort_pairs<LsgSortConfig<RB, BS, IPT>>(std::forward<Args>(args)...); }
template <unsigned RB, unsigned BS, unsigned IPT, class... Args>
static hipError_t lsg_segmented_sort_keys(Args&&... args) { return rocprim::segmented_radix_sort_keys<LsgSortConfig<RB, BS, IPT>>(std::forward<Args>(args)...); }

static bool count_in_load(const lsg_ctx* c) { return c->cal_enabled && c->n_ct >= 1 && c->n_ct <= 2 && c->n_cb > 0 && c->copy_stream; }

static int print_tile_hist(const lsg_ctx* c, uint32_t T) {
    std::vector<uint32_t> caps(T);
    LSG_HIP(hipMemcpy(caps.data(), c->d_tile_cap.p, (size_t)T * 4, hipMemcpyDeviceToHost));
    unsigned long long nt[8] = {0}, ne[8] = {0}; uint32_t mx = 0;
    const uint32_t lim[7] = {64, 256, 2048, 8192, 32768, 131072, 524288};
    for (uint32_t i = 0; i < T; ++i) { const uint32_t v = caps[i]; if (!v) continue; int k = 0; while (k < 7 && v > lim[k]) ++k; ++nt[k]; ne[k] += v; if (v > mx) mx = v; }
    for (int k = 0; k < 8; ++k) fprintf(stderr, "tiles <= %u: %llu tiles, %llu entries\n", k < 7 ? lim[k] : 0xffffffffu, nt[k], ne[k]);
    fprintf(stderr, "largest tile: %u entries\n", mx);
    return 0;
}

enum LoadRung { RUNG_WINDOWS = 1, RUNG_TILE_KEYS, RUNG_TILE_VALUES };

static int build_once(lsg_ctx* c, const uint16_t* events, int64_t n_events, const int64_t* seg_ev_off, const lsg_reads* src, int rung) {
    drop_store(c);
    hipStream_t st = c->stream;
    const int64_t S = c->rd.n_segs, R = c->rd.n_reads;
    const bool counts = count_in_load(c) && n_events >= 64 && n_events < (1ll << 39);
    const bool skip_store = c->cal_enabled && c->store_policy == LSG_STORE_SKIP_WHEN_COUNTED;
    const bool win = rung == RUNG_WINDOWS && skip_store && counts && n_events >= 128 &&
                     (c->events_layout == LSG_LAYOUT_PHASED || (c->hint_phased_events && c->hint_phased_events == (const void*)events)) && ((uintptr_t)events & 255u) == 0 && c->plp_window >= 128 &&
                     c->cal_params.min_bq >= 1 && c->cal_params.min_bq <= 255 && (c->n_tiles & 1u) == 0;
    const int wsh = win ? 1 : 0;
    c->wsh = wsh;
    const uint32_t T = c->n_tiles >> wsh;
    const auto t_wall = std::chrono::steady_clock::now();
    auto finish = [&]() {
        c->layout_build_ms = std::chrono::duration<double, std::milli>(std::chrono::steady_clock::now() - t_wall).count();
        c->tm_valid = true;
        return 0;
    };
    for (auto& v : c->build_ms) v = 0;
    c->st_min_mq = c->lf_min_mq; c->st_flag_exclude = c->lf_flag_exclude; c->st_ignore_orphans = c->lf_ignore_orphans;
    if (c->d_tile_cap.reserve(((size_t)T + 2) * 4) || c->d_tile_off.reserve(((size_t)T + 2) * 4) || c->d_scalars.reserve(512 * 8)) return -1;
    LSG_HIP(hipMemsetAsync(c->d_tile_cap.p, 0, ((size_t)T + 2) * 4, st));
    LSG_HIP(hipMemsetAsync(c->d_tile_off.p, 0, ((size_t)T + 2) * 4, st));
    if (S <= 0 || T == 0) { LSG_HIP(hipStreamSynchronize(st)); return finish(); }
    if (c->ws[WS_SEG_INFO].reserve(((size_t)S + 1) * 8)) return -1;
    LSG_HIP(hipMemsetAsync(c->d_scalars.p, 0, 64, st));
    BuildArgs a{};
    a.n_reads = R; a.n_segs = S; a.n_events = n_events;
    const lsg_reads& in = src ? *src : c->rd;
    a.read_tid = in.read_tid; a.read_flag = in.read_flag; a.read_mapq = in.read_mapq; a.read_cb = in.read_cb;
    a.seg_read = in.seg_read; a.seg_start = in.seg_start; a.seg_len = in.seg_len; a.seg_ev_off = seg_ev_off;
    a.tile_base = c->d_tile_base.as<uint32_t>(); a.contig_len = c->d_contig_len.as<int64_t>(); a.n_contigs = c->n_contigs; a.n_tiles = T;
    a.seg_info = c->ws[WS_SEG_INFO].as<uint2>(); a.tile_cap = c->d_tile_cap.as<uint32_t>();
    a.lf_min_mq = c->lf_min_mq; a.lf_flag_exclude = c->lf_flag_exclude; a.lf_ignore_orphans = c->lf_ignore_orphans;
    a.window = c->plp_window; c->st_window = c->plp_window; a.wsh = wsh;
    a.qhead = c->d_scalars.as<unsigned long long>(); a.bad = reinterpret_cast<uint32_t*>(c->d_scalars.as<unsigned long long>() + 2);
    a.n_ev = c->d_scalars.as<unsigned long long>() + 3;
    if (c->bt[BT_SPAN].reserve(((size_t)T + 2) * 4)) return -1;
    LSG_HIP(hipMemsetAsync(c->bt[BT_SPAN].p, 0, ((size_t)T + 2) * 4, st));
    a.span_diff = c->bt[BT_SPAN].as<int32_t>();
    uint32_t* d_small = reinterpret_cast<uint32_t*>(c->d_scalars.as<unsigned long long>() + 4);
    DevBuf& tmp = c->bt[BT_TMP];
    LSG_HIP(hipEventRecord(c->evb[0], st));
    unsigned g_seg = (unsigned)((S + 256 * SEG_U - 1) / (256 * SEG_U)); if (g_seg > (unsigned)(c->n_cus * 16)) g_seg = (unsigned)(c->n_cus * 16);
    unsigned g_bin = (unsigned)((S + 256 * BIN_SUPER - 1) / (256 * BIN_SUPER)); if (g_bin > (unsigned)(c->n_cus * 8)) g_bin = (unsigned)(c->n_cus * 8);
    if (c->bt[BT_PER_TILE].reserve(((size_t)T + 2) * 4)) return -1;
    LSG_HIP(hipMemsetAsync(c->bt[BT_PER_TILE].p, 0, ((size_t)T + 2) * 4, st));
    a.cap_diff = c->bt[BT_PER_TILE].as<int32_t>();
    hipLaunchKernelGGL(k_seg_static, dim3(g_seg), dim3(256), 0, st, a);
    if (c->bt[BT_NETILE].reserve(((size_t)T + 2) * 4) || c->tm[TM_BLK_OFF].reserve(((size_t)T + 2) * 4)) return -1;
    uint32_t* blk_off = c->tm[TM_BLK_OFF].as<uint32_t>();
    unsigned long long* d_sum = c->d_scalars.as<unsigned long long>() + 8;
    {
        size_t tb = 0;
        LSG_HIP(hipcub::DeviceReduce::Max(nullptr, tb, in.read_cb, reinterpret_cast<int32_t*>(d_small + 2), (int)(R > 0 ? R : 1), st));
        if (tmp.reserve(tb + 256 + 64 * 1024)) return -1;
        tb = tmp.cap;
        if (R > 0) LSG_HIP(hipcub::DeviceReduce::Max(tmp.p, tb, in.read_cb, reinterpret_cast<int32_t*>(d_small + 2), (int)R, st));
    }
    {
        if (c->d_cub_tmp.reserve(64 * 1024)) return -1;
        TtArgs ta{};
        ta.cap_diff = a.cap_diff; ta.span_diff = a.span_diff; ta.T = T;
        const uint64_t per = ((uint64_t)T + 1 + TT_MAX_CHUNKS - 1) / TT_MAX_CHUNKS;
        ta.chunk = (uint32_t)((per + TT_SUB - 1) / TT_SUB * TT_SUB);
        ta.n_chunks = (uint32_t)(((uint64_t)T + 1 + ta.chunk - 1) / ta.chunk);
        char* scratch = reinterpret_cast<char*>(c->d_cub_tmp.p);
        ta.agg1 = reinterpret_cast<TtAgg1*>(scratch); ta.agg2 = reinterpret_cast<TtAgg2*>(scratch + 16 * 1024); ta.in2 = reinterpret_cast<TtAgg2*>(scratch + 32 * 1024);
        ta.din = reinterpret_cast<int32_t*>(scratch + 48 * 1024);
        ta.cap = c->d_tile_cap.as<uint32_t>(); ta.tile_off = c->d_tile_off.as<uint32_t>(); ta.blk_off = blk_off; ta.netile = c->bt[BT_NETILE].as<uint32_t>();
        ta.d_small = d_small; ta.d_sum = d_sum;
        hipLaunchKernelGGL(k_tt_marks, dim3(ta.n_chunks), dim3(TT_THREADS), 0, st, ta);
        hipLaunchKernelGGL(k_tt_scan1, dim3(1), dim3(TT_MAX_CHUNKS), 0, st, ta);
        hipLaunchKernelGGL(k_tt_caps, dim3(ta.n_chunks), dim3(TT_THREADS), 0, st, ta);
        hipLaunchKernelGGL(k_tt_scan2, dim3(1), dim3(TT_MAX_CHUNKS), 0, st, ta);
        hipLaunchKernelGGL(k_tt_offsets, dim3(ta.n_chunks), dim3(TT_THREADS), 0, st, ta);
    }
    uint32_t total = 0, bad = 0, n_netile = 0, nblk = 0; int32_t max_cb = 0, max_live = 0;
    unsigned long long n_ev = 0, sum = 0;
    LSG_HIP(hipMemcpyAsync(c->h_pin, c->d_scalars.p, 9 * 8, hipMemcpyDeviceToHost, st));
    LSG_HIP(hipMemcpyAsync(c->h_pin + 16, blk_off + T, 4, hipMemcpyDeviceToHost, st));
    LSG_HIP(hipStreamSynchronize(st));
    {
        const unsigned long long* hp = c->h_pin;
        const uint32_t* hs = reinterpret_cast<const uint32_t*>(hp + 4);
        bad = (uint32_t)hp[2]; n_ev = hp[3]; n_netile = hs[1]; max_cb = R > 0 ? (int32_t)hs[2] : 0; max_live = (int32_t)hs[3]; sum = hp[8];
        nblk = (uint32_t)hp[16];
    }
    if (win && (bad & 4u) && !(bad & 3u)) return RUNG_TILE_KEYS;
    const int src_shift = !(bad & 4u) && ((uintptr_t)events & (wsh ? 255u : 127u)) == 0 ? 6 + wsh : 0;
    c->src_phased = src_shift != 0;
    if (bad & 2u) { set_error("lsg_load_reads: a segment's read index lies outside the read arrays"); return -2; }
    if (bad & 1u) { set_error("lsg_load_reads: a segment's event range lies outside the events array"); return -2; }
    if (sum >= 0x7FFFFFF0ull) { set_error("lsg_load_reads: %llu tile entries exceed the 31-bit entry index; load the reads in windows", sum); return -2; }
    total = (uint32_t)sum;
    const uint64_t N = total;
    c->tm_n = N; c->tm_events = (int64_t)n_ev;
    c->max_live_all = max_live > 0 ? max_live : 0;
    if (N == 0) return finish();
    if (getenv("LSG_TILE_HIST")) { if (int rc = print_tile_hist(c, T)) return rc; }
    int bits = 1; while (bits < 24 && (1ll << bits) <= (long long)max_cb) ++bits;
    DevBuf &key_a = c->bt[BT_KEY_A], &key_b = c->bt[BT_KEY_B], &val_a = c->bt[BT_VAL_A], &val_b = c->bt[BT_VAL_B];
    if ((n_events >> src_shift) >= (1ll << (52 - bits - 2 * wsh))) {
        set_error("lsg_load_reads: %lld events with %d-bit barcode ids do not fit the packed sort key (events < 2^%d): load the reads in windows", (long long)n_events, bits, 52 - bits + src_shift);
        return -2;
    }
    bool keys_only = rung <= RUNG_TILE_KEYS && skip_store && counts && (n_events >> src_shift) < (1ll << (50 - bits - 2 * wsh));
    bool cap_out = true;
    if (c->cal_enabled && c->cal_params.max_depth > 0 && c->max_live_all + 1 > (int64_t)c->cal_params.max_depth) {
        cap_out = false;
        if (count_in_load(c)) {
            LSG_HIP(hipStreamSynchronize(c->copy_stream));
            if (live_read_bound(c)) return -1;
            cap_out = c->max_live_reads + 1 <= (int64_t)c->cal_params.max_depth;
            if (!cap_out) {
                if (live_read_bound_exact(c)) return -1;
                cap_out = c->max_live_exact <= (int64_t)c->cal_params.max_depth;
            }
        }
    }
    if (keys_only) {
        const lsg_count_params& q = c->cal_params;
        if (q.min_mq != c->st_min_mq || q.flag_exclude != c->st_flag_exclude || (q.ignore_orphans != 0) != (c->st_ignore_orphans != 0)) keys_only = false;
        if (!cap_out) keys_only = false;
        for (int t = 0; t < c->n_contigs && keys_only; ++t) if (!c->ref_ptr[t]) keys_only = false;
    }
    if (win && !keys_only) return RUNG_TILE_KEYS;
    if (keys_only && getenv("LSG_TIMING")) fprintf(stderr, "[lsg] load: keys alone through the scatter and the sort (8 bytes an entry)%s\n", win ? ", entries binned by 128-position windows" : "");
    if (key_a.reserve(N * 8 + 16) || key_b.reserve(N * 8 + 16) || (!keys_only && (val_a.reserve(N * 4 + 16) || val_b.reserve(N * 4 + 16))) ||
        c->bt[BT_CURSOR].reserve(((size_t)T + 2) * 4)) return -1;
    a.cursor = c->bt[BT_CURSOR].as<uint32_t>(); a.key = key_a.as<uint64_t>(); a.rdv = keys_only ? nullptr : val_a.as<uint32_t>(); a.cb_bits = bits; a.src_shift = src_shift;
    LSG_HIP(hipMemcpyAsync(a.cursor, c->d_tile_off.p, ((size_t)T + 1) * 4, hipMemcpyDeviceToDevice, st));
    LSG_HIP(hipMemsetAsync(c->d_scalars.p, 0, 8, st));
    hipLaunchKernelGGL(k_bin, dim3(g_bin), dim3(BIN_THREADS), 0, st, a);
    LSG_HIP(hipEventRecord(c->evb[1], st));
    if (c->tm[TM_BLK_TILE].reserve(((size_t)nblk + 2) * 4)) return -1;
    bool blk_tiles_made = false;
    const bool lpt = n_netile > 1;
    const uint32_t* lpt_tiles = nullptr;
    auto blk_tiles = [&](hipStream_t s_) -> int {
        uint32_t* bt_ = c->tm[TM_BLK_TILE].as<uint32_t>();
        LSG_HIP(hipMemsetAsync(bt_, 0, (size_t)nblk * 4, s_));
        hipLaunchKernelGGL(k_tm_blk_mark, dim3((T + 255) / 256), dim3(256), 0, s_, c->d_tile_cap.as<uint32_t>(), blk_off, T, bt_);
        size_t tb = c->bt[BT_COPY_TMP].cap;
        LSG_HIP(hipcub::DeviceScan::InclusiveScan(c->bt[BT_COPY_TMP].p, tb, bt_, bt_, hipcub::Max(), (int)nblk, s_));
        LSG_HIP(hipEventRecord(c->ev_blk, s_));
        blk_tiles_made = true;
        return 0;
    };
    {
        hipStream_t bs = c->copy_stream;
        DevBuf& lk = c->bt[BT_LPT];
        const size_t lpt_pitch = ((size_t)n_netile + 64) & ~(size_t)63;
        if (lpt && lk.reserve(lpt_pitch * 4 * 3)) return -1;
        uint32_t* k_in = lk.as<uint32_t>(); uint32_t* k_out = k_in + lpt_pitch; uint32_t* t_out = k_out + lpt_pitch;
        uint32_t* bt_ = c->tm[TM_BLK_TILE].as<uint32_t>();
        size_t tb_lpt = 0, tb_blk = 0;
        if (lpt) LSG_HIP(hipcub::DeviceRadixSort::SortPairsDescending(nullptr, tb_lpt, k_in, k_out, c->bt[BT_NETILE].as<uint32_t>(), t_out, (int)n_netile, 0, 21, bs));
        LSG_HIP(hipcub::DeviceScan::InclusiveScan(nullptr, tb_blk, bt_, bt_, hipcub::Max(), (int)nblk, bs));
        size_t tb_sort2 = 0;
        if (n_netile) {
            if (keys_only) LSG_HIP((lsg_segmented_sort_keys<7, 256, 8>(nullptr, tb_sort2, (uint64_t*)nullptr, (uint64_t*)nullptr, (unsigned)N, (unsigned)n_netile, (uint32_t*)nullptr, (uint32_t*)nullptr, 0u, (unsigned)bits, bs, false)));
            else LSG_HIP((lsg_segmented_sort<7, 256, 8>(nullptr, tb_sort2, (uint64_t*)nullptr, (uint64_t*)nullptr, (uint32_t*)nullptr, (uint32_t*)nullptr, (unsigned)N, (unsigned)n_netile,
                                                        (uint32_t*)nullptr, (uint32_t*)nullptr, 0u, (unsigned)bits, bs, false)));
        }
        size_t tb_max = tb_lpt > tb_blk ? tb_lpt : tb_blk;
        if (tb_sort2 > tb_max) tb_max = tb_sort2;
        if (c->bt[BT_COPY_TMP].reserve(tb_max + 256)) return -1;
        void* scratch = c->bt[BT_COPY_TMP].p;
        if (lpt) {
            hipLaunchKernelGGL(k_tile_caps, dim3((n_netile + 255) / 256), dim3(256), 0, bs, c->bt[BT_NETILE].as<uint32_t>(), n_netile, c->d_tile_cap.as<uint32_t>(), k_in);
            size_t tb = c->bt[BT_COPY_TMP].cap;
            LSG_HIP(hipcub::DeviceRadixSort::SortPairsDescending(scratch, tb, k_in, k_out, c->bt[BT_NETILE].as<uint32_t>(), t_out, (int)n_netile, 0, 21, bs));
            LSG_HIP(hipEventRecord(c->ev_lpt, bs));
            lpt_tiles = t_out;
        }
        if (!skip_store) { if (int rc = blk_tiles(bs)) return rc; }
    }
    const bool tiles_planned = count_in_load(c);
    if (tiles_planned) {
        if (int rc = plan_tiles(c, c->copy_stream)) return rc;
        plan_finish_tiles(c);
    }
    if (n_netile) {
        const size_t seg_pitch = ((size_t)n_netile + 64) & ~(size_t)63;
        if (c->bt[BT_SEG_BEGIN].reserve(seg_pitch * 8) || c->bt[BT_SEG_END].reserve(seg_pitch * 8)) return -1;
        uint32_t* sb1 = c->bt[BT_SEG_BEGIN].as<uint32_t>(); uint32_t* se1 = c->bt[BT_SEG_END].as<uint32_t>();
        uint32_t* sb2 = sb1 + seg_pitch; uint32_t* se2 = se1 + seg_pitch;
        if (lpt) LSG_HIP(hipStreamWaitEvent(st, c->ev_lpt, 0));
        hipLaunchKernelGGL(k_seg_bounds, dim3((n_netile + 255) / 256), dim3(256), 0, st, lpt ? lpt_tiles : c->bt[BT_NETILE].as<uint32_t>(), n_netile, c->d_tile_off.as<uint32_t>(), sb1, se1, sb2, se2);
        LSG_HIP(hipEventRecord(c->ev_copy, st));
        size_t tb = 0;
        const bool big_blocks = N < (64ull << 20);
        auto sort = [&](void* tmp_p, size_t& tmp_n) {
            if (keys_only && big_blocks) return lsg_segmented_sort_keys<7, 512, 8>(tmp_p, tmp_n, key_a.as<uint64_t>(), key_b.as<uint64_t>(), (unsigned)N, (unsigned)n_netile, sb1, se1, 0u, (unsigned)bits, st, false);
            if (keys_only) return lsg_segmented_sort_keys<7, 256, 8>(tmp_p, tmp_n, key_a.as<uint64_t>(), key_b.as<uint64_t>(), (unsigned)N, (unsigned)n_netile, sb1, se1, 0u, (unsigned)bits, st, false);
            return lsg_segmented_sort<7, 256, 8>(tmp_p, tmp_n, key_a.as<uint64_t>(), key_b.as<uint64_t>(), val_a.as<uint32_t>(), val_b.as<uint32_t>(), (unsigned)N, (unsigned)n_netile,
                                                 sb1, se1, 0u, (unsigned)bits, st, false);
        };
        LSG_HIP(sort(nullptr, tb));
        if (tmp.reserve(tb + 256)) return -1;
        tb = tmp.cap;
        LSG_HIP(sort(tmp.p, tb));
        hipStream_t bs = c->copy_stream;
        LSG_HIP(hipStreamWaitEvent(bs, c->ev_copy, 0));
        size_t tb2 = c->bt[BT_COPY_TMP].cap;
        if (keys_only) LSG_HIP((lsg_segmented_sort_keys<7, 256, 8>(c->bt[BT_COPY_TMP].p, tb2, key_a.as<uint64_t>(), key_b.as<uint64_t>(), (unsigned)N, (unsigned)n_netile, sb2, se2, 0u, (unsigned)bits, bs, false)));
        else LSG_HIP((lsg_segmented_sort<7, 256, 8>(c->bt[BT_COPY_TMP].p, tb2, key_a.as<uint64_t>(), key_b.as<uint64_t>(), val_a.as<uint32_t>(), val_b.as<uint32_t>(), (unsigned)N, (unsigned)n_netile,
                                                    sb2, se2, 0u, (unsigned)bits, bs, false)));
        LSG_HIP(hipEventRecord(c->ev_lpt, bs));
        LSG_HIP(hipStreamWaitEvent(st, c->ev_lpt, 0));
    }
    LSG_HIP(hipEventRecord(c->evb[2], st));
    const uint64_t np = (uint64_t)nblk * 8;
    c->tm_np = np; c->tm_nblk = nblk;
    auto reserve_store = [&]() -> int {
    if (c->tm[TM_S0].reserve((np + 16) * 4) || c->tm[TM_B].reserve(np + 16) ||
        c->tm[TM_RD].reserve((np + 16) * 4) || c->tm[TM_META].reserve((np + 8 * (TM_GROUP + 1)) * 4) ||
        c->tm[TM_BLK_TILE].reserve(((size_t)nblk + 2) * 4) || c->tm[TM_EXT].reserve(((size_t)nblk + TM_GROUP + 2) * 2)) return -1;
    LSG_HIP(hipMemsetD32Async(reinterpret_cast<hipDeviceptr_t>(c->tm[TM_S0].as<uint32_t>() + np), (int)TM_PAD_S0, 16, st));
    LSG_HIP(hipMemsetAsync(c->tm[TM_B].as<uint8_t>() + np, 0, 16, st));
    if (c->tm[TM_STORE].cap < ((size_t)nblk + TM_GROUP) * 1024) {
        size_t mem_free = 0, mem_total = 0;
        if (hipMemGetInfo(&mem_free, &mem_total) == hipSuccess && ((size_t)nblk + TM_GROUP) * 1088 + (mem_total >> 5) > mem_free) {
            LSG_HIP(hipStreamSynchronize(st));
            key_a.release(); val_a.release(); c->ws[WS_SEG_INFO].release(); c->bt[BT_SPAN].release(); c->bt[BT_PEX].release(); c->bt[BT_OFFS].release();
        }
        if (c->tm[TM_STORE].reserve(((size_t)nblk + TM_GROUP) * 1024)) return -1;
    }
    return 0;
    };
    LSG_HIP(hipEventRecord(c->evb[3], st));
    bool fused = counts;
    if (fused) {
        const lsg_count_params& q = c->cal_params;
        if (q.min_mq < c->st_min_mq || (c->st_flag_exclude & ~q.flag_exclude) != 0 || (c->st_ignore_orphans && !q.ignore_orphans)) fused = false;
        if (fused && !cap_out) fused = false;
        for (int t = 0; t < c->n_contigs && fused; ++t) if (!c->ref_ptr[t]) fused = false;
    }
    const bool dbg = getenv("LSG_DEBUG_SYNC") != nullptr;
    auto stage = [&](const char* what) { if (dbg) { const hipError_t e = hipStreamSynchronize(st); fprintf(stderr, "[lsg] fused load: %s: %s\n", what, hipGetErrorString(e)); fflush(stderr); } };
    auto fused_plan = [&]() -> int {
        stage("scatter + sort + block tables");
        c->tm_np = np; c->tm_nblk = nblk;
        if (int rc = plan_jobs(c, false, key_b.as<uint64_t>(), bits)) return rc;
        stage("plan");
        return 0;
    };
    const GatherCountSrc gsrc{events, n_events, key_b.as<uint64_t>(), keys_only ? nullptr : val_b.as<uint32_t>(), bits, src_shift, wsh};
    bool planned = false;
    if (win && !fused) return RUNG_TILE_KEYS;
    if (keys_only && getenv("LSG_TEST_KEYS_ONLY_REFUSED")) return win ? RUNG_TILE_KEYS : RUNG_TILE_VALUES;
    if (fused && skip_store) {
        if (int rc = fused_plan()) return rc;
        planned = true;
        const int rc = run_gather_count(c, &c->cal_params, gsrc, true);
        LSG_HIP(hipStreamSynchronize(st));
        if (hipGetLastError() != hipSuccess) { set_error("lsg_load_reads: the count pass failed"); return -1; }
        if (rc < 0 && rc != -3) return rc;
        if (rc == 0) {
            plan_finish(c);
            LSG_HIP(hipStreamSynchronize(c->copy_stream));
            c->load_was_fused = true; c->counted_at_load = true; c->store_skipped = true;
            for (int i = 0; i < 4; ++i) { float ms = 0; if (hipEventElapsedTime(&ms, c->evb[i], c->evb[i + 1]) == hipSuccess) c->build_ms[i] = ms; }
            settle_temporaries(c);
            c->layout_build_ms = std::chrono::duration<double, std::milli>(std::chrono::steady_clock::now() - t_wall).count();
            return 0;
        }
        c->counted = false;
        fused = false;
    }
    if (win) return RUNG_TILE_KEYS;
    if (keys_only) return RUNG_TILE_VALUES;
    if (int rc = reserve_store()) return rc;
    if (!blk_tiles_made) {
        LSG_HIP(hipStreamSynchronize(c->copy_stream));
        if (int rc = blk_tiles(st)) return rc;
    }
    if (fused) {
        if (int rc = fused_plan()) return rc;
        c->tm_valid = true;
        int rc = run_gather_count(c, &c->cal_params, gsrc, false);
        LSG_HIP(hipStreamSynchronize(st));
        if (hipGetLastError() != hipSuccess) { c->tm_valid = false; set_error("lsg_load_reads: the fused gather + count pass failed"); return -1; }
        if (rc < 0 && rc != -3) { c->tm_valid = false; return rc; }
        plan_finish(c);
        c->load_was_fused = true;
        c->counted_at_load = rc == 0;
        if (rc) c->counted = false;
    } else {
    LSG_HIP(hipStreamWaitEvent(st, c->ev_blk, 0));
    const bool plan_early = c->n_ct > 0 && c->copy_stream && c->ev_copy && !planned;
    if (plan_early) LSG_HIP(hipEventRecord(c->ev_copy, st));
    {
        const dim3 grid((unsigned)(((((uint64_t)nblk + TMG_BLOCKS - 1) / TMG_BLOCKS + TMG_WAVES - 1) / TMG_WAVES + 7) / 8 * 8));
        hipLaunchKernelGGL(k_tm_gather, grid, dim3(TMG_WAVES * 64), 0, st,
                           events, n_events, key_b.as<uint64_t>(), val_b.as<uint32_t>(), bits, src_shift, c->d_tile_off.as<uint32_t>(), blk_off, c->tm[TM_BLK_TILE].as<uint32_t>(), nblk,
                           c->tm[TM_S0].as<uint32_t>(), c->tm[TM_B].as<uint8_t>(), c->tm[TM_RD].as<uint32_t>(),
                           c->tm[TM_STORE].as<uint4>(), c->tm[TM_EXT].as<uint16_t>());
    }
    LSG_HIP(hipEventRecord(c->evb[4], st));
    LSG_HIP(hipGetLastError());
    int plan_rc = 0;
    if (plan_early) {
        LSG_HIP(hipStreamWaitEvent(c->copy_stream, c->ev_copy, 0));
        plan_rc = tiles_planned ? 0 : plan_tiles(c, c->copy_stream);
        if (!plan_rc) {
            c->tm_np = np; c->tm_nblk = nblk;
            plan_rc = plan_jobs(c, false);
        }
    }
    LSG_HIP(hipStreamSynchronize(st));
    if (plan_early) LSG_HIP(hipStreamSynchronize(c->copy_stream));
    if (plan_rc) return plan_rc;
    if (plan_early || planned) plan_finish(c);
    }
    for (int i = 0; i < 4; ++i) { float ms = 0; if (hipEventElapsedTime(&ms, c->evb[i], c->evb[i + 1]) == hipSuccess) c->build_ms[i] = ms; }
    settle_temporaries(c);
    if (getenv("LSG_TIMING"))
        fprintf(stderr, "[lsg] tile store: %llu entries, %u blocks (%.2f GB): capacities + scatter %.2f, sort %.2f, fill %.2f, gather %.2f ms\n",
                (unsigned long long)N, nblk, (double)nblk * 1024 / 1e9, c->build_ms[0], c->build_ms[1], c->build_ms[2], c->build_ms[3]);
    return finish();
}

int build_store(lsg_ctx* c, const uint16_t* events, int64_t n_events, const int64_t* seg_ev_off, const lsg_reads* src) {
    int rc = build_once(c, events, n_events, seg_ev_off, src, RUNG_WINDOWS);
    while (rc > 0) {
        LSG_HIP(hipStreamSynchronize(c->stream)); LSG_HIP(hipStreamSynchronize(c->copy_stream));
        if (getenv("LSG_TIMING"))
            fprintf(stderr, rc == RUNG_TILE_KEYS ? "[lsg] load: not a load for 128-position windows after all, starting again by tiles\n"
                                                 : "[lsg] load: the count from keys alone was not made, loading again with values\n");
        rc = build_once(c, events, n_events, seg_ev_off, src, rc);
    }
    return rc;
}

constexpr uint32_t TM_CHUNK_WORK = 4096, TM_JOB_W0 = 32;

__global__ void k_tm_tiles(const uint32_t* cap, uint32_t n_tiles, int n_ct, uint32_t job_tgt, uint32_t H, uint32_t* ne, uint32_t* nj, uint32_t* slabs, uint32_t* multi) {
    const uint32_t t = blockIdx.x * blockDim.x + threadIdx.x;
    if (t > n_tiles) return;
    const uint32_t n = t < n_tiles ? cap[t] : 0u;
    const uint32_t j = n == 0 ? 0u : (n <= job_tgt ? 1u : (n + job_tgt - 1) / job_tgt);
    ne[t] = n ? H : 0u; nj[t] = j; slabs[t] = j > 1 ? j * (uint32_t)n_ct * H : 0u; multi[t] = j > 1 ? H : 0u;
}
struct RunSrc { const uint32_t* s0; const uint64_t* key; uint32_t cbm; };
__device__ __forceinline__ void tm_make_job(const RunSrc& rs, uint64_t base, uint32_t off, uint32_t n, uint32_t J, uint32_t j, uint32_t w0, uint32_t slab, uint32_t tile, int2 geom,
                                            TmJob* out, uint32_t* n_wide) {
    auto starts = [&](uint32_t x) -> bool {
        if (!rs.key) return (rs.s0[base + x] & TM_RUNSTART) != 0;
        return x == 0 || (((uint32_t)rs.key[off + x] ^ (uint32_t)rs.key[off + x - 1]) & rs.cbm) != 0;
    };
    auto cut = [&](uint32_t x) -> uint32_t { while (x < n && !starts(x)) ++x; return x < n ? x : n; };
    const uint32_t e0 = j == 0 ? 0u : cut((uint32_t)(((uint64_t)n * j) / J));
    uint32_t e1 = j + 1 == J ? n : cut((uint32_t)(((uint64_t)n * (j + 1)) / J));
    if (e1 < e0) e1 = e0;
    TmJob jb;
    jb.e0 = (uint32_t)(base + e0); jb.e1 = (uint32_t)(base + e1); jb.w0 = w0;
    jb.slab = J > 1 ? slab : 0xFFFFFFFFu; jb.nj = J; jb.cnt = n; jb.tile = tile;
    jb.base = (uint32_t)base; jb.off = off; jb.tstart = geom.x; jb.tid = geom.y & 0xffffff;
    uint32_t mid = e1;
    if (e1 - e0 >= 64u) { mid = cut(e0 + (e1 - e0) / 2u); if (mid > e1) mid = e1; }
    jb.emid = (uint32_t)(base + mid);
    if (e1 - e0 > (uint32_t)TM_JOB_LIMIT) { jb.nj |= TMJ_WIDE; atomicAdd(n_wide, 1u); }
    *out = jb;
}
__global__ void k_tm_jobs(const uint32_t* tile_base, int n_contigs, int n_ct, int wsh, RunSrc rs, const uint32_t* tile_off, const uint32_t* cap, const uint32_t* blk_off, const uint32_t* ne_off,
                          const uint32_t* nj, const uint32_t* job_off, const uint32_t* slab_off, const uint32_t* multi_off, uint32_t n_tiles, TmJob* jobs,
                          uint32_t* ne_units, int2* ne_geom, uint32_t* ne_nslot, uint32_t* ne_acc, uint32_t* multi, uint32_t* n_wide) {
    const uint32_t t = blockIdx.x * blockDim.x + threadIdx.x;
    if (t >= n_tiles) return;
    const uint32_t n = cap[t];
    if (!n) return;
    const uint32_t J = nj[t], ord = ne_off[t];
    const uint64_t base = (uint64_t)blk_off[t] * 8;
    const uint32_t tile0 = t << wsh;
    int tid = 0;
    { int lo = 0, hi = n_contigs; while (hi - lo > 1) { const int mid = (lo + hi) >> 1; if (tile_base[mid] <= tile0) lo = mid; else hi = mid; } tid = lo; }
    const int32_t tstart = (int32_t)((tile0 - tile_base[tid]) << 6);
    for (uint32_t h = 0; h < (1u << wsh); ++h)
    for (int ct = 0; ct < n_ct; ++ct) {
        const uint32_t w = (ord + h) * (uint32_t)n_ct + ct;
        ne_units[w] = (tile0 + h) * (uint32_t)n_ct + ct;
        ne_geom[w] = make_int2(tstart + 64 * (int32_t)h, tid | (ct << 24));
        ne_nslot[w] = J;
        ne_acc[w] = J > 1 ? slab_off[t] + (h * (uint32_t)n_ct + (uint32_t)ct) * J : 0u;
        if (J > 1) multi[(multi_off[t] + h) * (uint32_t)n_ct + ct] = w;
    }
    if (J > 1) return;
    tm_make_job(rs, base, tile_off[t], n, 1u, 0u, ord * (uint32_t)n_ct, 0xFFFFFFFFu, t, make_int2(tstart, tid), jobs + job_off[t], n_wide);
}
__global__ __launch_bounds__(64) void k_tm_jobs_multi(int n_ct, int wsh, RunSrc rs, const uint32_t* tile_off, const uint32_t* cap, const uint32_t* blk_off, const uint32_t* ne_off, const uint32_t* nj,
                                                      const uint32_t* job_off, const uint32_t* slab_off, const uint32_t* multi, const uint32_t* ne_units, const int2* ne_geom, uint32_t n_mt,
                                                      TmJob* jobs, uint32_t* n_wide) {
    const uint32_t i = blockIdx.x;
    if (i >= n_mt) return;
    const uint32_t w = multi[((size_t)i << wsh) * (uint32_t)n_ct], t = (ne_units[w] / (uint32_t)n_ct) >> wsh;
    const uint32_t n = cap[t], J = nj[t];
    const int2 geom = ne_geom[w];
    const uint64_t base = (uint64_t)blk_off[t] * 8;
    for (uint32_t j = threadIdx.x; j < J; j += 64u)
        tm_make_job(rs, base, tile_off[t], n, J, j, ne_off[t] * (uint32_t)n_ct, slab_off[t] + j, t, geom, jobs + job_off[t] + j, n_wide);
}
struct TmJobWork {
    const TmJob* jobs;
    __host__ __device__ uint32_t operator()(const uint32_t& j) const { return jobs[j].e1 - jobs[j].e0 + TM_JOB_W0; }
};
__global__ void k_tm_chunks(const uint32_t* pex, uint32_t njobs, uint32_t chunk_work, uint32_t* chunk_start, uint32_t* n_chunks) {
    const uint32_t j = blockIdx.x * blockDim.x + threadIdx.x;
    if (j >= njobs) return;
    const uint32_t ck = pex[j] / chunk_work;
    const int64_t prev = j ? (int64_t)(pex[j - 1] / chunk_work) : -1;
    for (int64_t k = prev + 1; k <= (int64_t)ck; ++k) chunk_start[k] = j;
    if (j == njobs - 1) { chunk_start[ck + 1] = njobs; *n_chunks = ck + 1; }
}

static int plan_tiles(lsg_ctx* c, hipStream_t st) {
    const uint32_t T = c->n_tiles >> c->wsh;
    const uint64_t N = c->tm_n;
    DevBuf &per_tile = c->bt[BT_PER_TILE], &offs = c->bt[BT_OFFS];
    if (per_tile.reserve((size_t)(T + 2) * 4 * 4) || offs.reserve((size_t)(T + 2) * 4 * 4 + 64)) return -1;
    uint32_t* ne = per_tile.as<uint32_t>(); uint32_t* nj = ne + (T + 2); uint32_t* slabs = nj + (T + 2); uint32_t* multi = slabs + (T + 2);
    uint32_t* ne_off = offs.as<uint32_t>(); uint32_t* job_off = ne_off + (T + 2); uint32_t* slab_off = job_off + (T + 2); uint32_t* multi_off = slab_off + (T + 2);
    uint32_t* d_misc = multi_off + (T + 2);
    uint32_t job_tgt = TM_JOB_TGT;
    { const uint64_t per = N / ((uint64_t)c->n_cus * 14 * 4); if (per < job_tgt) job_tgt = (uint32_t)(per < 768 ? 768 : per); }
    hipLaunchKernelGGL(k_tm_tiles, dim3((T + 256) / 256), dim3(256), 0, st, c->d_tile_cap.as<uint32_t>(), T, c->n_ct, job_tgt, 1u << c->wsh, ne, nj, slabs, multi);
    SCAN_U32(ne, ne_off, T + 1); SCAN_U32(nj, job_off, T + 1); SCAN_U32(slabs, slab_off, T + 1); SCAN_U32(multi, multi_off, T + 1);
    LSG_HIP(hipMemsetAsync(d_misc, 0, 8, st));
    uint32_t* srcs[4] = {ne_off, job_off, slab_off, multi_off};
    for (int i = 0; i < 4; ++i) LSG_HIP(hipMemcpyAsync(&c->plan1_tot[i], srcs[i] + T, 4, hipMemcpyDeviceToHost, st));
    LSG_HIP(hipStreamSynchronize(st));
    const uint32_t n_net = c->plan1_tot[0], njobs = c->plan1_tot[1], n_mt = c->plan1_tot[3];
    const size_t n_ne = (size_t)n_net * (size_t)c->n_ct, n_multi = (size_t)n_mt * (size_t)c->n_ct;
    if (c->tm[TM_JOBS].reserve(((size_t)njobs + 1) * sizeof(TmJob)) || c->tm[TM_NE_UNITS].reserve((n_ne + 2) * 4) || c->tm[TM_NE_GEOM].reserve((n_ne + 2) * 8) ||
        c->tm[TM_NE_NSLOT].reserve((n_ne + 2) * 4) || c->tm[TM_NE_ACC].reserve((n_ne + 2) * 4) || c->tm[TM_MULTI].reserve((n_multi + 2) * 4)) return -1;
    LSG_HIP(hipMemsetAsync(c->tm[TM_NE_NSLOT].p, 0, (n_ne + 2) * 4, st));
    LSG_HIP(hipMemsetAsync(c->tm[TM_NE_ACC].p, 0, (n_ne + 2) * 4, st));
    LSG_HIP(hipStreamSynchronize(st));
    c->plan1_n_ct = c->n_ct;
    return 0;
}

static int plan_jobs(lsg_ctx* c, bool finish, const uint64_t* skey, int cb_bits) {
    hipStream_t st = c->stream;
    const RunSrc rs{c->tm[TM_S0].as<uint32_t>(), skey, skey ? (1u << cb_bits) - 1u : 0u};
    const uint32_t T = c->n_tiles >> c->wsh;
    DevBuf &per_tile = c->bt[BT_PER_TILE], &offs = c->bt[BT_OFFS];
    uint32_t* nj = per_tile.as<uint32_t>() + (T + 2);
    uint32_t* ne_off = offs.as<uint32_t>(); uint32_t* job_off = ne_off + (T + 2); uint32_t* slab_off = job_off + (T + 2); uint32_t* multi_off = slab_off + (T + 2);
    uint32_t* d_misc = multi_off + (T + 2);
    const uint32_t* tot = c->plan1_tot;
    const uint32_t njobs = tot[1], n_mt = tot[3];
    hipLaunchKernelGGL(k_tm_jobs, dim3((T + 255) / 256), dim3(256), 0, st, c->d_tile_base.as<uint32_t>(), c->n_contigs, c->n_ct, c->wsh, rs, c->d_tile_off.as<uint32_t>(),
                       c->d_tile_cap.as<uint32_t>(), c->tm[TM_BLK_OFF].as<uint32_t>(), ne_off, nj, job_off, slab_off, multi_off, T,
                       c->tm[TM_JOBS].as<TmJob>(), c->tm[TM_NE_UNITS].as<uint32_t>(), c->tm[TM_NE_GEOM].as<int2>(), c->tm[TM_NE_NSLOT].as<uint32_t>(),
                       c->tm[TM_NE_ACC].as<uint32_t>(), c->tm[TM_MULTI].as<uint32_t>(), d_misc);
    if (n_mt) hipLaunchKernelGGL(k_tm_jobs_multi, dim3(n_mt >> c->wsh), dim3(64), 0, st, c->n_ct, c->wsh, rs, c->d_tile_off.as<uint32_t>(), c->d_tile_cap.as<uint32_t>(), c->tm[TM_BLK_OFF].as<uint32_t>(),
                                 ne_off, nj, job_off, slab_off, c->tm[TM_MULTI].as<uint32_t>(), c->tm[TM_NE_UNITS].as<uint32_t>(), c->tm[TM_NE_GEOM].as<int2>(), n_mt >> c->wsh, c->tm[TM_JOBS].as<TmJob>(), d_misc);
    {
        DevBuf& pex = c->bt[BT_PEX];
        const uint64_t total_work = c->tm_np + (uint64_t)njobs * TM_JOB_W0;
        const uint64_t cw = total_work / ((uint64_t)c->n_cus * 14 * 6);
        const uint32_t chunk_work = (uint32_t)(cw < 256 ? 256 : (cw > TM_CHUNK_WORK ? TM_CHUNK_WORK : cw));
        if (pex.reserve(((size_t)njobs + 2) * 4) || c->tm[TM_CHUNKS].reserve(((size_t)(total_work / chunk_work) + 4) * 4)) return -1;
        hipcub::CountingInputIterator<uint32_t> iota(0);
        TmJobWork wf{c->tm[TM_JOBS].as<TmJob>()};
        hipcub::TransformInputIterator<uint32_t, TmJobWork, hipcub::CountingInputIterator<uint32_t>> it(iota, wf);
        SCAN_U32(it, pex.as<uint32_t>(), njobs);
        hipLaunchKernelGGL(k_tm_chunks, dim3((njobs + 255) / 256), dim3(256), 0, st, pex.as<uint32_t>(), njobs, chunk_work, c->tm[TM_CHUNKS].as<uint32_t>(), d_misc + 1);
    }
    LSG_HIP(hipMemcpyAsync(c->plan_misc, d_misc, 8, hipMemcpyDeviceToHost, st));
    c->d_plan_misc = d_misc;
    LSG_HIP(hipGetLastError());
    if (finish) LSG_HIP(hipStreamSynchronize(st));
    return 0;
}

static void plan_finish_tiles(lsg_ctx* c) {
    const uint32_t* tot = c->plan1_tot;
    c->tm_njobs = tot[1];
    c->tm_n_ne = (uint32_t)((size_t)tot[0] * (size_t)c->n_ct); c->tm_n_multi = (uint32_t)((size_t)tot[3] * (size_t)c->n_ct); c->tm_n_slabs = tot[2];
}
static void plan_finish(lsg_ctx* c) {
    plan_finish_tiles(c);
    c->tm_nchunks = c->plan_misc[1]; c->tm_n_wide = c->plan_misc[0];
    c->plan_n_ct = c->n_ct;
    if (getenv("LSG_TIMING")) {
        std::vector<TmJob> jobs(c->tm_njobs);
        uint32_t longest = 0;
        if (c->tm_njobs && hipMemcpy(jobs.data(), c->tm[TM_JOBS].p, (size_t)c->tm_njobs * sizeof(TmJob), hipMemcpyDeviceToHost) != hipSuccess) { (void)hipGetLastError(); return; }
        for (const TmJob& jb : jobs) if (!(jb.nj & TMJ_WIDE) && jb.e1 - jb.e0 > longest) longest = jb.e1 - jb.e0;
        fprintf(stderr, "[lsg] plan: %u jobs, %u multi-job tiles, %u wide, longest packed job %u entries\n", c->tm_njobs, c->plan1_tot[3], c->tm_n_wide, longest);
    }
}

int ensure_plan(lsg_ctx* c) {
    if (!c->tm_valid) { set_error("lsg_pileup_count: no reads loaded"); return -2; }
    if (c->plan_n_ct == c->n_ct) return 0;
    c->plan_n_ct = 0;
    c->tm_njobs = c->tm_nchunks = c->tm_n_ne = c->tm_n_multi = c->tm_n_slabs = c->tm_n_wide = 0;
    if (c->tm_nblk == 0) { c->plan_n_ct = c->n_ct; return 0; }
    if (c->plan1_n_ct != c->n_ct) { if (int rc = plan_tiles(c, c->stream)) return rc; }
    if (int rc = plan_jobs(c, true)) return rc;
    plan_finish(c);
    return 0;
}

}
```

Baseline: 3.525 billion.

## Defer read-array copies, self-clear tile marks, and cache barcode max across builds

Device-to-device copies of the read arrays are deferred and issued on the copy stream only after the first build kernel launches, with the barcode max reduction run on that stream from the source array and cached across rebuild rungs. The tile mark kernels now zero the diff arrays as they read them, so the per-build memsets can be skipped when the buffers are unchanged, tracked through a generation counter. The scan kernel also writes the bin cursor directly, which removes a separate copy and memset. The aim is to cut serial memsets, copies and a CUB reduction from the load critical path. The cost is extra state that must stay consistent, such as the clean-marks tracking and the destructor that issues any copies still pending.

Result: no change. 3.533 billion (median of 4 runs) (+0.2%).

```diff
diff --git a/longsom_amd/csrc/lsg_api.hip b/longsom_amd/csrc/lsg_api.hip
--- a/longsom_amd/csrc/lsg_api.hip
+++ b/longsom_amd/csrc/lsg_api.hip
@@ -1,6 +1,7 @@
 #include "lsg_ctx.h"
 #include <cstdarg>
 #include <cstring>
+#include <type_traits>
 
 namespace lsg {
 static thread_local char g_err[512] = "";
@@ -45,11 +46,11 @@
 int run_sf4(lsg_ctx* c, int64_t items, const uint32_t* k, const uint32_t* n, double al, double be, int32_t* out, double* raw);
 
 template <class T>
-static int put(lsg_ctx* c, DevBuf& buf, const T*& dst, const T* src, int64_t n, int on_device, hipStream_t st = nullptr) {
+static int put(lsg_ctx* c, DevBuf& buf, const T*& dst, const T* src, int64_t n, int on_device) {
     if (n <= 0 || !src) { dst = nullptr; return 0; }
     if (src == buf.as<T>()) { dst = src; return 0; }
     if (buf.reserve((size_t)n * sizeof(T))) return -1;
-    LSG_HIP(hipMemcpyAsync(buf.p, src, (size_t)n * sizeof(T), on_device ? hipMemcpyDeviceToDevice : hipMemcpyHostToDevice, st ? st : c->stream));
+    LSG_HIP(hipMemcpyAsync(buf.p, src, (size_t)n * sizeof(T), on_device ? hipMemcpyDeviceToDevice : hipMemcpyHostToDevice, c->stream));
     dst = buf.as<T>();
     return 0;
 }
@@ -82,7 +83,7 @@
     lsg_ctx* c = new lsg_ctx();
     c->device = device_id;
     { hipDeviceProp_t prop; if (hipGetDeviceProperties(&prop, device_id) == hipSuccess && prop.multiProcessorCount > 0) c->n_cus = prop.multiProcessorCount; }
-    if (hipStreamCreateWithFlags(&c->copy_stream, hipStreamNonBlocking) != hipSuccess || hipEventCreateWithFlags(&c->ev_copy, hipEventDisableTiming) != hipSuccess || hipEventCreateWithFlags(&c->ev_blk, hipEventDisableTiming) != hipSuccess || hipEventCreateWithFlags(&c->ev_lpt, hipEventDisableTiming) != hipSuccess ||
+    if (hipStreamCreateWithFlags(&c->copy_stream, hipStreamNonBlocking) != hipSuccess || hipEventCreateWithFlags(&c->ev_copy, hipEventDisableTiming) != hipSuccess || hipEventCreateWithFlags(&c->ev_cb, hipEventDisableTiming) != hipSuccess || hipEventCreateWithFlags(&c->ev_blk, hipEventDisableTiming) != hipSuccess || hipEventCreateWithFlags(&c->ev_lpt, hipEventDisableTiming) != hipSuccess ||
         hipStreamCreateWithFlags(&c->own_stream, hipStreamNonBlocking) != hipSuccess) {
         set_error("lsg_create: hipStreamCreate failed"); delete c; return -1;
     }
@@ -126,6 +127,7 @@
     if (c->own_stream) (void)hipStreamDestroy(c->own_stream);
     if (c->copy_stream) (void)hipStreamDestroy(c->copy_stream);
     if (c->ev_copy) (void)hipEventDestroy(c->ev_copy);
+    if (c->ev_cb) (void)hipEventDestroy(c->ev_cb);
     if (c->ev_blk) (void)hipEventDestroy(c->ev_blk);
     if (c->ev_lpt) (void)hipEventDestroy(c->ev_lpt);
     if (c->h_pin) (void)hipHostFree(c->h_pin);
@@ -319,24 +321,45 @@
     if (in.n_segs > 0 && (!in.seg_read || !in.seg_start || !in.seg_len || !in.seg_ev_off)) { c->rd = lsg_reads{}; set_error("lsg_load_reads: NULL segment array"); return -2; }
     if (in.n_events > 0 && !in.events) { c->rd = lsg_reads{}; set_error("lsg_load_reads: NULL events array"); return -2; }
     hipStream_t cs = nullptr;
+    c->lc = LoadCopies{};
     if (d && !c->keep_reads) {
-        LSG_HIP(hipEventRecord(c->ev_copy, c->stream));
-        LSG_HIP(hipStreamWaitEvent(c->copy_stream, c->ev_copy, 0));
         cs = c->copy_stream;
-    }
-    if (put(c, c->b_read_tid, c->rd.read_tid, in.read_tid, in.n_reads, d, cs) ||
-        put(c, c->b_read_pos, c->rd.read_pos, in.read_pos, in.n_reads, d, cs) ||
-        put(c, c->b_read_flag, c->rd.read_flag, in.read_flag, in.n_reads, d, cs) ||
-        put(c, c->b_read_mapq, c->rd.read_mapq, in.read_mapq, in.n_reads, d, cs) ||
-        put(c, c->b_read_cb, c->rd.read_cb, in.read_cb, in.n_reads, d, cs) ||
-        put(c, c->b_seg_read, c->rd.seg_read, in.seg_read, in.n_segs, d, cs) ||
-        put(c, c->b_seg_start, c->rd.seg_start, in.seg_start, in.n_segs, d, cs) ||
-        put(c, c->b_seg_len, c->rd.seg_len, in.seg_len, in.n_segs, d, cs)) { if (cs) (void)hipStreamSynchronize(cs); c->rd = lsg_reads{}; return -1; }
+        int k = 0;
+        auto defer = [&](DevBuf& buf, auto*& dst, auto* src, int64_t n) -> int {
+            LoadCopies::Range& g = c->lc.r[k++];
+            g = LoadCopies::Range{nullptr, nullptr, 0};
+            if (n <= 0 || !src) { dst = nullptr; return 0; }
+            if (src == buf.as<std::remove_pointer_t<decltype(src)>>()) { dst = src; return 0; }
+            if (buf.reserve((size_t)n * sizeof(*src))) return -1;
+            g = LoadCopies::Range{buf.p, src, (unsigned long long)n * sizeof(*src)};
+            dst = buf.as<std::remove_pointer_t<decltype(src)>>();
+            return 0;
+        };
+        if (defer(c->b_read_tid, c->rd.read_tid, in.read_tid, in.n_reads) ||
+            defer(c->b_read_pos, c->rd.read_pos, in.read_pos, in.n_reads) ||
+            defer(c->b_read_flag, c->rd.read_flag, in.read_flag, in.n_reads) ||
+            defer(c->b_read_mapq, c->rd.read_mapq, in.read_mapq, in.n_reads) ||
+            defer(c->b_read_cb, c->rd.read_cb, in.read_cb, in.n_reads) ||
+            defer(c->b_seg_read, c->rd.seg_read, in.seg_read, in.n_segs) ||
+            defer(c->b_seg_start, c->rd.seg_start, in.seg_start, in.n_segs) ||
+            defer(c->b_seg_len, c->rd.seg_len, in.seg_len, in.n_segs)) { c->lc = LoadCopies{}; c->rd = lsg_reads{}; return -1; }
+        c->lc.cb_src = in.read_cb;
+        c->lc.pending = true;
+    } else if (put(c, c->b_read_tid, c->rd.read_tid, in.read_tid, in.n_reads, d) ||
+        put(c, c->b_read_pos, c->rd.read_pos, in.read_pos, in.n_reads, d) ||
+        put(c, c->b_read_flag, c->rd.read_flag, in.read_flag, in.n_reads, d) ||
+        put(c, c->b_read_mapq, c->rd.read_mapq, in.read_mapq, in.n_reads, d) ||
+        put(c, c->b_read_cb, c->rd.read_cb, in.read_cb, in.n_reads, d) ||
+        put(c, c->b_seg_read, c->rd.seg_read, in.seg_read, in.n_segs, d) ||
+        put(c, c->b_seg_start, c->rd.seg_start, in.seg_start, in.n_segs, d) ||
+        put(c, c->b_seg_len, c->rd.seg_len, in.seg_len, in.n_segs, d)) { c->rd = lsg_reads{}; return -1; }
     const uint16_t* ev = in.events; const int64_t* evo = in.seg_ev_off;
     const bool staged = !d || c->keep_reads;
     if (staged && (put(c, c->b_seg_ev_off, evo, in.seg_ev_off, in.n_segs, d) || put(c, c->b_events, ev, in.events, in.n_events, d))) { c->rd = lsg_reads{}; return -1; }
     if (staged && in.events && c->hint_phased_events == (const void*)in.events) c->hint_phased_events = ev;
-    const int rc = lsg::build_store(c, ev, in.n_events, evo, cs ? &in : nullptr);
+    int rc = lsg::build_store(c, ev, in.n_events, evo, cs ? &in : nullptr);
+    if (!rc && c->lc.pending) rc = lsg::issue_load_copies(c);
+    c->lc.pending = false;
     if (cs) LSG_HIP(hipStreamSynchronize(cs));
     if (rc) { c->rd = lsg_reads{}; lsg::drop_store(c); return rc; }
     if (c->keep_reads) { c->rd.events = ev; c->rd.seg_ev_off = evo; }
diff --git a/longsom_amd/csrc/lsg_ctx.h b/longsom_amd/csrc/lsg_ctx.h
--- a/longsom_amd/csrc/lsg_ctx.h
+++ b/longsom_amd/csrc/lsg_ctx.h
@@ -38,17 +38,29 @@
 struct DevBuf {
     void* p = nullptr;
     size_t cap = 0;
+    uint32_t gen = 0;
     int reserve(size_t bytes) {
         if (bytes <= cap) return 0;
         if (p) { (void)hipFree(p); p = nullptr; cap = 0; }
         const size_t slack = bytes / 16 < ((size_t)64 << 20) ? bytes / 16 : ((size_t)64 << 20);
         size_t want = bytes + slack + 256;
+        ++gen;
         LSG_HIP(hipMalloc(&p, want));
         cap = want;
         return 0;
     }
-    void release() { if (p) (void)hipFree(p); p = nullptr; cap = 0; }
+    void release() { if (p) (void)hipFree(p); p = nullptr; cap = 0; ++gen; }
     template <class T> T* as() const { return reinterpret_cast<T*>(p); }
+};
+
+constexpr int LC_RANGES = 8;
+struct LoadCopies {
+    struct Range { void* dst; const void* src; unsigned long long bytes; } r[LC_RANGES];
+    const int32_t* cb_src = nullptr;
+    bool pending = false;
+    bool ordered = false;
+    bool cb_max_known = false;
+    int32_t cb_max = 0;
 };
 
 struct PosSet { DevBuf keys; int64_t n = 0; };
@@ -131,6 +143,7 @@
 struct lsg_ctx;
 namespace lsg {
 int build_store(lsg_ctx* c, const uint16_t* events, int64_t n_events, const int64_t* seg_ev_off, const lsg_reads* src = nullptr);
+int issue_load_copies(lsg_ctx* c);
 int ensure_plan(lsg_ctx* c);
 void drop_store(lsg_ctx* c);
 int live_read_bound(lsg_ctx* c);
@@ -150,6 +163,7 @@
     hipStream_t own_stream = nullptr;
     hipStream_t copy_stream = nullptr;
     hipEvent_t ev_copy = nullptr;
+    hipEvent_t ev_cb = nullptr;
     hipEvent_t ev_blk = nullptr;
     hipEvent_t ev_lpt = nullptr;
     hipEvent_t ev[6] = {nullptr, nullptr, nullptr, nullptr, nullptr, nullptr};
@@ -172,6 +186,7 @@
     lsg_reads rd{};
     lsg::DevBuf b_read_tid, b_read_pos, b_read_flag, b_read_mapq, b_read_cb;
     lsg::DevBuf b_seg_read, b_seg_start, b_seg_len, b_seg_ev_off, b_events;
+    lsg::LoadCopies lc;
     int32_t plp_window = 50000, st_window = 50000;
     int32_t lf_min_mq = 0, lf_ignore_orphans = 0; uint32_t lf_flag_exclude = 0;
     int32_t st_min_mq = 0, st_ignore_orphans = 0; uint32_t st_flag_exclude = 0;
@@ -182,6 +197,7 @@
     lsg::DevBuf d_tile_cap, d_tile_off;
     lsg::DevBuf tm[lsg::TM_NBUF];
     lsg::DevBuf bt[18];
+    size_t marks_clean = 0; uint32_t marks_gen[2] = {0, 0};
     uint64_t tm_n = 0;
     int64_t tm_events = 0;
     uint64_t tm_np = 0;
diff --git a/longsom_amd/csrc/store.hip b/longsom_amd/csrc/store.hip
--- a/longsom_amd/csrc/store.hip
+++ b/longsom_amd/csrc/store.hip
@@ -384,10 +384,11 @@
 struct TtAgg1 { int32_t d, s, smax, pad; };
 struct TtAgg2 { unsigned long long c; uint32_t b, ne; };
 struct TtArgs {
-    const int32_t* cap_diff; const int32_t* span_diff; uint32_t T; uint32_t chunk;
+    int32_t* cap_diff; int32_t* span_diff; uint32_t T; uint32_t chunk;
     uint32_t n_chunks;
     TtAgg1* agg1; int32_t* din; TtAgg2* agg2; TtAgg2* in2;
     uint32_t* cap; uint32_t* tile_off; uint32_t* blk_off; uint32_t* netile;
+    uint32_t* cursor;
     uint32_t* d_small; unsigned long long* d_sum;
 };
 template <int NT, class V>
@@ -413,6 +414,8 @@
         int32_t d[4], sp[4];
 #pragma unroll
         for (int k = 0; k < 4; ++k) { const bool in = i0 + k < hi; d[k] = in ? a.cap_diff[i0 + k] : 0; sp[k] = in && a.span_diff ? a.span_diff[i0 + k] : 0; }
+#pragma unroll
+        for (int k = 0; k < 4; ++k) if (i0 + k < hi && a.span_diff && sp[k] != 0) a.span_diff[i0 + k] = 0;
         int32_t ds = d[0] + d[1] + d[2] + d[3];
         int32_t r = 0, m = INT32_MIN;
 #pragma unroll
@@ -460,6 +463,8 @@
         int32_t d[4];
 #pragma unroll
         for (int k = 0; k < 4; ++k) d[k] = i0 + k < hi ? a.cap_diff[i0 + k] : 0;
+#pragma unroll
+        for (int k = 0; k < 4; ++k) if (i0 + k < hi && d[k] != 0) a.cap_diff[i0 + k] = 0;
         int32_t tot; const int32_t ex = tt_wg_exscan<TT_THREADS>(d[0] + d[1] + d[2] + d[3], tot, sh);
         int32_t r = run + ex;
 #pragma unroll
@@ -480,6 +485,7 @@
         TtAgg2 g{0, 0, 0};
         for (int w = 0; w < TT_THREADS / 64; ++w) { g.c += sh_c[w]; g.b += sh_b[w]; g.ne += sh_n[w]; }
         a.agg2[blockIdx.x] = g;
+        if (blockIdx.x == 0) a.cap[a.T + 1] = 0;
     }
 }
 __global__ __launch_bounds__(TT_MAX_CHUNKS) void k_tt_scan2(TtArgs a) {
@@ -513,13 +519,14 @@
 #pragma unroll
         for (int k = 0; k < 4; ++k) {
             if (i0 + k < hi) {
-                a.tile_off[i0 + k] = ec; a.blk_off[i0 + k] = eb;
+                a.tile_off[i0 + k] = ec; a.blk_off[i0 + k] = eb; a.cursor[i0 + k] = ec;
                 if (nv[k]) a.netile[en] = i0 + k;
             }
             ec += cv[k]; eb += bv[k]; en += nv[k];
         }
         crun += tc; brun += tb; nrun += tn;
     }
+    if (blockIdx.x == 0 && threadIdx.x == 0) a.tile_off[a.T + 1] = 0;
 }
 constexpr uint32_t SORT_LARGE = 256;
 __global__ void k_seg_bounds(const uint32_t* netile, uint32_t n, const uint32_t* tile_off, uint32_t* begin, uint32_t* end, uint32_t* begin2, uint32_t* end2) {
@@ -630,7 +637,7 @@
         LSG_HIP(hipcub::DeviceScan::ExclusiveSum(c->d_cub_tmp.p, tb_, (in), (out), (int)(n), st));       \
     } while (0)
 
-enum { BT_KEY_A = 0, BT_KEY_B, BT_VAL_A, BT_VAL_B, BT_PEX, BT_NETILE, BT_SEG_BEGIN, BT_SEG_END, BT_TMP, BT_PER_TILE, BT_OFFS, BT_SPAN, BT_CURSOR, BT_LPT, BT_COPY_TMP, BT_N };
+enum { BT_KEY_A = 0, BT_KEY_B, BT_VAL_A, BT_VAL_B, BT_PEX, BT_NETILE, BT_SEG_BEGIN, BT_SEG_END, BT_TMP, BT_PER_TILE, BT_OFFS, BT_SPAN, BT_CURSOR, BT_LPT, BT_COPY_TMP, BT_CAP_DIFF, BT_N };
 
 void drop_store(lsg_ctx* c) {
     c->tm_valid = false; c->plan_n_ct = 0; c->plan1_n_ct = 0; c->tm_n = 0; c->tm_events = 0; c->tm_np = 0; c->tm_nblk = 0; c->tm_njobs = 0; c->tm_nchunks = 0;
@@ -646,6 +653,43 @@
     if (hipMemGetInfo(&mem_free, &mem_total) != hipSuccess) return;
     const bool tight = c->store_skipped ? mem_free < mem_total / 4 : (held > mem_total / 8 || mem_free < mem_total / 8);
     if (tight) { for (auto& b : c->bt) b.release(); c->ws[WS_SEG_INFO].release(); c->plan1_n_ct = 0; }
+}
+
+constexpr int CBM_THREADS = 256;
+__global__ __launch_bounds__(CBM_THREADS) void k_cb_max(const int32_t* cb, long long n_reads, uint32_t* cb_max) {
+    __shared__ int32_t s_max[CBM_THREADS / 64];
+    const long long stride = (long long)gridDim.x * CBM_THREADS;
+    int32_t mx = INT32_MIN;
+    for (long long i = (long long)blockIdx.x * CBM_THREADS + threadIdx.x; i < n_reads; i += stride) { const int32_t x = cb[i]; mx = x > mx ? x : mx; }
+    for (int o = 32; o > 0; o >>= 1) { const int32_t u = __shfl_down(mx, o); mx = u > mx ? u : mx; }
+    if ((threadIdx.x & 63) == 0) s_max[threadIdx.x >> 6] = mx;
+    __syncthreads();
+    if (threadIdx.x == 0) {
+        for (int w = 1; w < CBM_THREADS / 64; ++w) mx = s_max[w] > mx ? s_max[w] : mx;
+        if ((long long)blockIdx.x * CBM_THREADS < n_reads) atomicMax(cb_max, (uint32_t)mx ^ 0x80000000u);
+    }
+}
+static int order_load_copies(lsg_ctx* c) {
+    LSG_HIP(hipEventRecord(c->ev_copy, c->stream));
+    LSG_HIP(hipStreamWaitEvent(c->copy_stream, c->ev_copy, 0));
+    c->lc.ordered = true;
+    return 0;
+}
+int issue_load_copies(lsg_ctx* c) {
+    if (!c->lc.pending) return 0;
+    c->lc.pending = false;
+    if (!c->lc.ordered) { if (int rc = order_load_copies(c)) return rc; }
+    for (const LoadCopies::Range& r : c->lc.r)
+        if (r.bytes) LSG_HIP(hipMemcpyAsync(r.dst, r.src, (size_t)r.bytes, hipMemcpyDeviceToDevice, c->copy_stream));
+    return 0;
+}
+static int issue_cb_max(lsg_ctx* c, const int32_t* cb, int64_t n_reads, uint32_t* word) {
+    const long long need = (n_reads + CBM_THREADS * 8 - 1) / (CBM_THREADS * 8);
+    const unsigned grid = (unsigned)(need < (long long)c->n_cus * 2 ? (need < 1 ? 1 : need) : (long long)c->n_cus * 2);
+    hipLaunchKernelGGL(k_cb_max, dim3(grid), dim3(CBM_THREADS), 0, c->copy_stream, cb, (long long)n_reads, word);
+    LSG_HIP(hipGetLastError());
+    LSG_HIP(hipEventRecord(c->ev_cb, c->copy_stream));
+    return 0;
 }
 
 static int plan_tiles(lsg_ctx* c, hipStream_t st);
@@ -677,6 +721,7 @@
 
 static int build_once(lsg_ctx* c, const uint16_t* events, int64_t n_events, const int64_t* seg_ev_off, const lsg_reads* src, int rung) {
     drop_store(c);
+    struct CopiesOnExit { lsg_ctx* c; ~CopiesOnExit() { (void)issue_load_copies(c); } } copies_on_exit{c};
     hipStream_t st = c->stream;
     const int64_t S = c->rd.n_segs, R = c->rd.n_reads;
     const bool counts = count_in_load(c) && n_events >= 64 && n_events < (1ll << 39);
@@ -696,9 +741,12 @@
     for (auto& v : c->build_ms) v = 0;
     c->st_min_mq = c->lf_min_mq; c->st_flag_exclude = c->lf_flag_exclude; c->st_ignore_orphans = c->lf_ignore_orphans;
     if (c->d_tile_cap.reserve(((size_t)T + 2) * 4) || c->d_tile_off.reserve(((size_t)T + 2) * 4) || c->d_scalars.reserve(512 * 8)) return -1;
-    LSG_HIP(hipMemsetAsync(c->d_tile_cap.p, 0, ((size_t)T + 2) * 4, st));
-    LSG_HIP(hipMemsetAsync(c->d_tile_off.p, 0, ((size_t)T + 2) * 4, st));
-    if (S <= 0 || T == 0) { LSG_HIP(hipStreamSynchronize(st)); return finish(); }
+    if (S <= 0 || T == 0) {
+        LSG_HIP(hipMemsetAsync(c->d_tile_cap.p, 0, ((size_t)T + 2) * 4, st));
+        LSG_HIP(hipMemsetAsync(c->d_tile_off.p, 0, ((size_t)T + 2) * 4, st));
+        LSG_HIP(hipStreamSynchronize(st));
+        return finish();
+    }
     if (c->ws[WS_SEG_INFO].reserve(((size_t)S + 1) * 8)) return -1;
     LSG_HIP(hipMemsetAsync(c->d_scalars.p, 0, 64, st));
     BuildArgs a{};
@@ -712,22 +760,30 @@
     a.window = c->plp_window; c->st_window = c->plp_window; a.wsh = wsh;
     a.qhead = c->d_scalars.as<unsigned long long>(); a.bad = reinterpret_cast<uint32_t*>(c->d_scalars.as<unsigned long long>() + 2);
     a.n_ev = c->d_scalars.as<unsigned long long>() + 3;
-    if (c->bt[BT_SPAN].reserve(((size_t)T + 2) * 4)) return -1;
-    LSG_HIP(hipMemsetAsync(c->bt[BT_SPAN].p, 0, ((size_t)T + 2) * 4, st));
+    if (c->bt[BT_SPAN].reserve(((size_t)T + 2) * 4) || c->bt[BT_CAP_DIFF].reserve(((size_t)T + 2) * 4)) return -1;
+    if (c->marks_gen[0] != c->bt[BT_SPAN].gen || c->marks_gen[1] != c->bt[BT_CAP_DIFF].gen || c->marks_clean < (size_t)T + 2) {
+        LSG_HIP(hipMemsetAsync(c->bt[BT_SPAN].p, 0, ((size_t)T + 2) * 4, st));
+        LSG_HIP(hipMemsetAsync(c->bt[BT_CAP_DIFF].p, 0, ((size_t)T + 2) * 4, st));
+    }
+    c->marks_clean = 0;
     a.span_diff = c->bt[BT_SPAN].as<int32_t>();
     uint32_t* d_small = reinterpret_cast<uint32_t*>(c->d_scalars.as<unsigned long long>() + 4);
     DevBuf& tmp = c->bt[BT_TMP];
     LSG_HIP(hipEventRecord(c->evb[0], st));
     unsigned g_seg = (unsigned)((S + 256 * SEG_U - 1) / (256 * SEG_U)); if (g_seg > (unsigned)(c->n_cus * 16)) g_seg = (unsigned)(c->n_cus * 16);
     unsigned g_bin = (unsigned)((S + 256 * BIN_SUPER - 1) / (256 * BIN_SUPER)); if (g_bin > (unsigned)(c->n_cus * 8)) g_bin = (unsigned)(c->n_cus * 8);
-    if (c->bt[BT_PER_TILE].reserve(((size_t)T + 2) * 4)) return -1;
-    LSG_HIP(hipMemsetAsync(c->bt[BT_PER_TILE].p, 0, ((size_t)T + 2) * 4, st));
-    a.cap_diff = c->bt[BT_PER_TILE].as<int32_t>();
+    a.cap_diff = c->bt[BT_CAP_DIFF].as<int32_t>();
+    if (c->bt[BT_NETILE].reserve(((size_t)T + 2) * 4) || c->tm[TM_BLK_OFF].reserve(((size_t)T + 2) * 4) || c->bt[BT_CURSOR].reserve(((size_t)T + 2) * 4) ||
+        c->d_cub_tmp.reserve(64 * 1024)) return -1;
+    const bool copies_now = src && c->lc.pending;
+    if (copies_now) { if (int rc = order_load_copies(c)) return rc; }
     hipLaunchKernelGGL(k_seg_static, dim3(g_seg), dim3(256), 0, st, a);
-    if (c->bt[BT_NETILE].reserve(((size_t)T + 2) * 4) || c->tm[TM_BLK_OFF].reserve(((size_t)T + 2) * 4)) return -1;
+    const bool cb_from_copy = copies_now && !c->lc.cb_max_known && R > 0 && c->lc.cb_src;
+    if (copies_now) { if (int rc = issue_load_copies(c)) return rc; }
+    if (cb_from_copy) { if (int rc = issue_cb_max(c, c->lc.cb_src, R, d_small + 2)) return rc; }
     uint32_t* blk_off = c->tm[TM_BLK_OFF].as<uint32_t>();
     unsigned long long* d_sum = c->d_scalars.as<unsigned long long>() + 8;
-    {
+    if (!c->lc.cb_max_known && !cb_from_copy) {
         size_t tb = 0;
         LSG_HIP(hipcub::DeviceReduce::Max(nullptr, tb, in.read_cb, reinterpret_cast<int32_t*>(d_small + 2), (int)(R > 0 ? R : 1), st));
         if (tmp.reserve(tb + 256 + 64 * 1024)) return -1;
@@ -735,7 +791,6 @@
         if (R > 0) LSG_HIP(hipcub::DeviceReduce::Max(tmp.p, tb, in.read_cb, reinterpret_cast<int32_t*>(d_small + 2), (int)R, st));
     }
     {
-        if (c->d_cub_tmp.reserve(64 * 1024)) return -1;
         TtArgs ta{};
         ta.cap_diff = a.cap_diff; ta.span_diff = a.span_diff; ta.T = T;
         const uint64_t per = ((uint64_t)T + 1 + TT_MAX_CHUNKS - 1) / TT_MAX_CHUNKS;
@@ -745,23 +800,27 @@
         ta.agg1 = reinterpret_cast<TtAgg1*>(scratch); ta.agg2 = reinterpret_cast<TtAgg2*>(scratch + 16 * 1024); ta.in2 = reinterpret_cast<TtAgg2*>(scratch + 32 * 1024);
         ta.din = reinterpret_cast<int32_t*>(scratch + 48 * 1024);
         ta.cap = c->d_tile_cap.as<uint32_t>(); ta.tile_off = c->d_tile_off.as<uint32_t>(); ta.blk_off = blk_off; ta.netile = c->bt[BT_NETILE].as<uint32_t>();
-        ta.d_small = d_small; ta.d_sum = d_sum;
+        ta.d_small = d_small; ta.d_sum = d_sum; ta.cursor = c->bt[BT_CURSOR].as<uint32_t>();
         hipLaunchKernelGGL(k_tt_marks, dim3(ta.n_chunks), dim3(TT_THREADS), 0, st, ta);
         hipLaunchKernelGGL(k_tt_scan1, dim3(1), dim3(TT_MAX_CHUNKS), 0, st, ta);
         hipLaunchKernelGGL(k_tt_caps, dim3(ta.n_chunks), dim3(TT_THREADS), 0, st, ta);
         hipLaunchKernelGGL(k_tt_scan2, dim3(1), dim3(TT_MAX_CHUNKS), 0, st, ta);
         hipLaunchKernelGGL(k_tt_offsets, dim3(ta.n_chunks), dim3(TT_THREADS), 0, st, ta);
+        c->marks_clean = (size_t)T + 2; c->marks_gen[0] = c->bt[BT_SPAN].gen; c->marks_gen[1] = c->bt[BT_CAP_DIFF].gen;
     }
     uint32_t total = 0, bad = 0, n_netile = 0, nblk = 0; int32_t max_cb = 0, max_live = 0;
     unsigned long long n_ev = 0, sum = 0;
+    if (cb_from_copy) LSG_HIP(hipStreamWaitEvent(st, c->ev_cb, 0));
     LSG_HIP(hipMemcpyAsync(c->h_pin, c->d_scalars.p, 9 * 8, hipMemcpyDeviceToHost, st));
     LSG_HIP(hipMemcpyAsync(c->h_pin + 16, blk_off + T, 4, hipMemcpyDeviceToHost, st));
     LSG_HIP(hipStreamSynchronize(st));
     {
         const unsigned long long* hp = c->h_pin;
         const uint32_t* hs = reinterpret_cast<const uint32_t*>(hp + 4);
-        bad = (uint32_t)hp[2]; n_ev = hp[3]; n_netile = hs[1]; max_cb = R > 0 ? (int32_t)hs[2] : 0; max_live = (int32_t)hs[3]; sum = hp[8];
+        bad = (uint32_t)hp[2]; n_ev = hp[3]; n_netile = hs[1]; max_live = (int32_t)hs[3]; sum = hp[8];
         nblk = (uint32_t)hp[16];
+        if (!c->lc.cb_max_known) { c->lc.cb_max = R > 0 ? (int32_t)(cb_from_copy ? hs[2] ^ 0x80000000u : hs[2]) : 0; c->lc.cb_max_known = true; }
+        max_cb = c->lc.cb_max;
     }
     if (win && (bad & 4u) && !(bad & 3u)) return RUNG_TILE_KEYS;
     const int src_shift = !(bad & 4u) && ((uintptr_t)events & (wsh ? 255u : 127u)) == 0 ? 6 + wsh : 0;
@@ -786,6 +845,7 @@
     if (c->cal_enabled && c->cal_params.max_depth > 0 && c->max_live_all + 1 > (int64_t)c->cal_params.max_depth) {
         cap_out = false;
         if (count_in_load(c)) {
+            if (int rc = issue_load_copies(c)) return rc;
             LSG_HIP(hipStreamSynchronize(c->copy_stream));
             if (live_read_bound(c)) return -1;
             cap_out = c->max_live_reads + 1 <= (int64_t)c->cal_params.max_depth;
@@ -803,11 +863,8 @@
     }
     if (win && !keys_only) return RUNG_TILE_KEYS;
     if (keys_only && getenv("LSG_TIMING")) fprintf(stderr, "[lsg] load: keys alone through the scatter and the sort (8 bytes an entry)%s\n", win ? ", entries binned by 128-position windows" : "");
-    if (key_a.reserve(N * 8 + 16) || key_b.reserve(N * 8 + 16) || (!keys_only && (val_a.reserve(N * 4 + 16) || val_b.reserve(N * 4 + 16))) ||
-        c->bt[BT_CURSOR].reserve(((size_t)T + 2) * 4)) return -1;
+    if (key_a.reserve(N * 8 + 16) || key_b.reserve(N * 8 + 16) || (!keys_only && (val_a.reserve(N * 4 + 16) || val_b.reserve(N * 4 + 16)))) return -1;
     a.cursor = c->bt[BT_CURSOR].as<uint32_t>(); a.key = key_a.as<uint64_t>(); a.rdv = keys_only ? nullptr : val_a.as<uint32_t>(); a.cb_bits = bits; a.src_shift = src_shift;
-    LSG_HIP(hipMemcpyAsync(a.cursor, c->d_tile_off.p, ((size_t)T + 1) * 4, hipMemcpyDeviceToDevice, st));
-    LSG_HIP(hipMemsetAsync(c->d_scalars.p, 0, 8, st));
     hipLaunchKernelGGL(k_bin, dim3(g_bin), dim3(BIN_THREADS), 0, st, a);
     LSG_HIP(hipEventRecord(c->evb[1], st));
     if (c->tm[TM_BLK_TILE].reserve(((size_t)nblk + 2) * 4)) return -1;
```
